# tanm-sys/forge-ec

Hardware: AMD Instinct MI355X
Metric: secp256k1-var scalar-muls/sec (batched, bit-exact vs CPU oracle on the parity sample) (higher is better)
Workload: dtype u32

## Files before the change

### forge_ec_amd/build.py

```python
import hashlib
import os
import subprocess
import sys

HERE = os.path.dirname(os.path.abspath(__file__))
SRC_DIR = os.path.join(HERE, "csrc")
OBJ_DIR = os.path.join(SRC_DIR, "_obj")
SO = os.path.join(HERE, "libfecgpu.so")
STAMP = SO + ".sha256"
SOURCES = ["fecgpu.hip", "canon.hip", "kernels_p256.hip", "kernels_ed.hip", "kernels_secp.hip", "kernels_codec.hip", "kernels_ecdsa.hip"]
HEADERS = ["coop.hpp", "sched_lf.hpp", "limbs.hpp", "staging.hpp", "host_ctx.hpp", "secp256k1.hpp", "p256.hpp", "ed25519.hpp",
           "canon_curves.hpp", "canon_kernels.hpp", "field_asm.inc", "kernels.hpp", "cu_split.hpp", os.path.join("..", "..", "include", "fecgpu.h"),
           os.path.join("..", "..", "include", "fecgpu_canon.h")]
FLAGS = ["--offload-arch=gfx950", "-O3", "-std=c++17", "-fPIC"]


def source_hash():
    h = hashlib.sha256(" ".join(FLAGS).encode())
    for rel in SOURCES + HEADERS:
        with open(os.path.join(SRC_DIR, rel), "rb") as f:
            h.update(rel.encode() + b"\0" + f.read())
    return h.hexdigest()


def up_to_date():
    try:
        return os.path.exists(SO) and open(STAMP).read().strip() == source_hash()
    except OSError:
        return False


DECLARATION_ONLY = ("kernels.hpp",)


def tu_closure_hash(src, kernel_code_only=False):
    import re
    seen, todo = [], [src]
    while todo:
        rel = todo.pop()
        if rel in seen or not os.path.exists(os.path.join(SRC_DIR, rel)) or (kernel_code_only and rel in DECLARATION_ONLY):
            continue
        seen.append(rel)
        with open(os.path.join(SRC_DIR, rel), "r") as f:
            todo += re.findall(r'^\s*#\s*include\s+"([^"/]+)"', f.read(), flags=re.M)
    h = hashlib.sha256(" ".join(FLAGS).encode())
    for rel in sorted(seen):
        with open(os.path.join(SRC_DIR, rel), "rb") as f:
            h.update(rel.encode() + b"\0" + f.read())
    return h.hexdigest()


WORKLOAD_TU = {"secp256k1-var": "kernels_secp.hip", "secp256k1-fixed": "kernels_secp.hip",
               "p256-var": "kernels_p256.hip", "p256-fixed": "kernels_p256.hip",
               "ed25519-var": "kernels_ed.hip", "ed25519-fixed": "kernels_ed.hip", "secp256k1-double": "kernels_secp.hip"}


def _tu_hash(src):
    return tu_closure_hash(src)


def build(force=False, verbose=False):
    if not force and up_to_date():
        return SO
    hipcc = os.environ.get("HIPCC", "/opt/rocm/bin/hipcc")
    os.makedirs(OBJ_DIR, exist_ok=True)
    for stale in (SO, STAMP):
        if os.path.exists(stale):
            os.remove(stale)
    jobs, objs, stamps = [], [], []
    for src in SOURCES:
        obj = os.path.join(OBJ_DIR, src.replace(".hip", ".o"))
        objs.append(obj)
        ostamp, want = obj + ".sha256", _tu_hash(src)
        try:
            if not force and os.path.exists(obj) and open(ostamp).read().strip() == want:
                continue
        except OSError:
            pass
        if os.path.exists(ostamp):
            os.remove(ostamp)
        cmd = [hipcc] + FLAGS + ["-c", os.path.join(SRC_DIR, src), "-o", obj]
        if verbose:
            print(" ".join(cmd), flush=True)
        jobs.append((cmd, subprocess.Popen(cmd)))
        stamps.append((ostamp, want))
    failed = [(cmd, proc.returncode) for cmd, proc in jobs if proc.wait() != 0]
    if failed:
        raise subprocess.CalledProcessError(failed[0][1], failed[0][0])
    for ostamp, want in stamps:
        with open(ostamp, "w") as f:
            f.write(want + "\n")
    cmd = [hipcc, "--offload-arch=gfx950", "-shared", "-fPIC", "-o", SO] + objs
    if verbose:
        print(" ".join(cmd), flush=True)
    subprocess.check_call(cmd)
    with open(STAMP, "w") as f:
        f.write(source_hash() + "\n")
    return SO


if __name__ == "__main__":
    print(build(force="--force" in sys.argv, verbose=True))
```

### forge_ec_amd/csrc/kernels_secp.hip

```cpp
#include <hip/hip_runtime.h>

#include "../../include/fecgpu.h"
#include "secp256k1.hpp"
#include "staging.hpp"
#include "kernels.hpp"

namespace fecgpu {

namespace {

FEC_DEV secp::pt ld3(const u32* l, int stride) {
  secp::pt p;
  FEC_UNROLL for (int i = 0; i < 8; ++i) {
    p.x.w[i] = l[i * stride];
    p.y.w[i] = l[(8 + i) * stride];
    p.z.w[i] = l[(16 + i) * stride];
  }
  return p;
}
FEC_DEV void st3(u32* l, int stride, const secp::pt& p) {
  FEC_UNROLL for (int i = 0; i < 8; ++i) {
    l[i * stride] = p.x.w[i];
    l[(8 + i) * stride] = p.y.w[i];
    l[(16 + i) * stride] = p.z.w[i];
  }
}

FEC_DEV fe ldc(const u32* l, int c) {
  fe a;
  FEC_UNROLL for (int i = 0; i < 8; ++i) a.w[i] = l[(8 * c + i) * TPB];
  return a;
}

FEC_DEV secp::pt padd_slots(const u32* lp, const u32* lq, lmask& need_double) {
  using namespace secp;
  fe z1s, z1c, z2s, z2c;
  lmask maybe;
  {
    const fe z1 = ldc(lp, 2);
    maybe = lanes_where(z1.w[0] == 0u);
    z1s = sqr(z1);
    z1c = mul(z1s, z1);
  }
  __builtin_amdgcn_sched_barrier(0);
  {
    const fe z2 = ldc(lq, 2);
    maybe |= lanes_where(z2.w[0] == 0u);
    z2s = sqr(z2);
    z2c = mul(z2s, z2);
  }
  __builtin_amdgcn_sched_barrier(0);
  const fe u1 = mul(ldc(lp, 0), z2s);
  const fe u2 = mul(ldc(lq, 0), z1s);
  __builtin_amdgcn_sched_barrier(0);
  const fe s1 = mul(ldc(lp, 1), z2c);
  const fe s2 = mul(ldc(lq, 1), z1c);
  __builtin_amdgcn_sched_barrier(0);
  lmask ueq = 0, seq = 0;
  if (__builtin_expect(lanes_where(u1.w[0] == u2.w[0]) != 0, 0)) {
    ueq = fe_eq(u1, u2);
    seq = fe_eq(s1, s2);
  }
  const fe h = sub(u2, u1);
  const fe r = sub(s2, s1);
  const fe h2 = sqr(h);
  const fe h3 = mul(h2, h);
  const fe u1h2 = mul(u1, h2);
  pt o;
  o.x = sub(sub(sub(sqr(r), h3), u1h2), u1h2);
  o.y = sub(mul(r, sub(u1h2, o.x)), mul(s1, h3));
  o.z = mul(mul(h, ldc(lp, 2)), ldc(lq, 2));
  need_double = 0;
  if (__builtin_expect((maybe | ueq) != 0, 0)) {
    const pt p = ld3(lp, TPB), q = ld3(lq, TPB);
    const lmask idp = is_identity(p), idq = is_identity(q);
    o = pt_select(o, identity(), ueq & ~seq);
    o = pt_select(o, p, idq);
    o = pt_select(o, q, idp);
    need_double = ueq & seq & ~idp & ~idq;
  }
  return o;
}

}

template <int MODE>
__global__ __launch_bounds__(TPB, 3) void k_secp_mul(const u32* __restrict__ scalars,
                                                  const u32* __restrict__ points,
                                                  u32* __restrict__ out, size_t n,
                                                  const u32* __restrict__ prefix, int wbits) {
  __shared__ u32 lds[48 * TPB];
  const int valid = block_valid(n);
  const size_t first = (size_t)blockIdx.x * TPB;
  const int e = threadIdx.x;
  if (MODE == 0) stage_in<24>(lds, points + first * 24, valid);
  __syncthreads();
  if (e < valid) {
    const size_t g = first + e;
    const u32* kg = scalars + g * 8;
    lmask early = 0;
    u32* const slot0 = lds + e;
    int i0 = 0, i1 = 256;
    if (MODE != 3) {
      u32 any = 0;
      FEC_UNROLL for (int i = 0; i < 8; ++i) any |= kg[i];
      early = lanes_where(any == 0);
    }
    if (MODE == 2) early |= secp::is_identity(ld3(points, 1));
    if (MODE == 2 || MODE == 3) {
      const u32 idx = MODE == 3 ? (u32)(g >> 1) : __builtin_bswap32(kg[0]) >> (32 - wbits);
      const uint4* row = reinterpret_cast<const uint4*>(prefix + (size_t)idx * 48);
      FEC_UNROLL for (int q = 0; q < 12; ++q) {
        const uint4 x = row[q];
        slot0[(4 * q + 0) * TPB] = x.x;
        slot0[(4 * q + 1) * TPB] = x.y;
        slot0[(4 * q + 2) * TPB] = x.z;
        slot0[(4 * q + 3) * TPB] = x.w;
      }
      i0 = MODE == 3 ? 0 : wbits;
      if (MODE == 3) i1 = 1;
    } else {
      const secp::pt r1 = MODE != 0 ? ld3(points, 1) : ld3(lds + e, TPB);
      early |= secp::is_identity(r1);
      st3(slot0, TPB, secp::identity());
      st3(slot0 + 24 * TPB, TPB, r1);
    }
    u32 kword = MODE == 3 ? 0u : kg[i0 >> 5];
#pragma unroll 1
    for (int i = i0; i < i1; ++i) {
      u32 b;
      if (MODE == 3) {
        b = (u32)g & 1u;
      } else {
        if ((i & 31) == 0) kword = kg[i >> 5];
        const int sh = (((i >> 3) & 3) << 3) + 7 - (i & 7);
        b = (kword >> sh) & 1u;
      }
      lmask nd;
      secp::pt s = padd_slots(slot0, slot0 + 24 * TPB, nd);
      if (__builtin_expect(nd != 0, 0)) {
        secp::pt d0 = secp::pdouble(ld3(slot0, TPB));
        s = secp::pt_select(s, d0, nd);
      }
      u32* const slot_d = slot0 + b * (24u * TPB);
      u32* const slot_s = slot0 + (b ^ 1u) * (24u * TPB);
      const secp::pt din = ld3(slot_d, TPB);
      st3(slot_s, TPB, s);
      st3(slot_d, TPB, secp::pdouble(din));
    }
    if (MODE != 3) {
      const secp::pt r0 = secp::pt_select(ld3(slot0, TPB), secp::identity(), early);
      st3(slot0, TPB, r0);
    }
  }
  __syncthreads();
  if (MODE == 3) stage_out<48>(out + first * 48, lds, valid);
  else stage_out<24>(out + first * 24, lds, valid);
}

void secp_launch_mul(const SchedEnv& env, bool fixed, const u32* scalars, const u32* points, u32* out, size_t n, hipStream_t s) {
  const unsigned grid = (unsigned)((n + TPB - 1) / TPB);
  const int w = (int)env.gen_prefix_bits[FEC_SECP256K1];
  if (fixed && w > 0 && points == env.gen[FEC_SECP256K1] && env.gen_prefix[FEC_SECP256K1] != nullptr)
    hipLaunchKernelGGL((k_secp_mul<2>), dim3(grid), dim3(TPB), 0, s, scalars, points, out, n, env.gen_prefix[FEC_SECP256K1], w);
  else if (fixed) hipLaunchKernelGGL((k_secp_mul<1>), dim3(grid), dim3(TPB), 0, s, scalars, points, out, n, (const u32*)nullptr, 0);
  else hipLaunchKernelGGL((k_secp_mul<0>), dim3(grid), dim3(TPB), 0, s, scalars, points, out, n, (const u32*)nullptr, 0);
}

void secp_prefix_level_launch(const u32* parent, u32* child, size_t child_entries, hipStream_t s) {
  hipLaunchKernelGGL((k_secp_mul<3>), dim3((unsigned)((child_entries + TPB - 1) / TPB)), dim3(TPB), 0, s, (const u32*)nullptr,
                     (const u32*)nullptr, child, child_entries, parent, 0);
}

}
```

### forge_ec_amd/csrc/secp256k1.hpp

```cpp
#pragma once
#include "limbs.hpp"

namespace fecgpu {
namespace secp {

#define FEC_SECP_C 0x3d1, 1, 0, 0, 0, 0, 0, 0
#define FEC_SECP_P 0xfffffc2f, -2, -1, -1, -1, -1, -1, -1

FEC_DEV fe csub_p(const fe& v) {
  fe w;
  lmask ov;
  FEC_ADDK256(w, v, ov, FEC_SECP_C);
  return fe_select(v, w, ov);
}
FEC_DEV lmask maybe_ge_p(const fe& v) {
  u32 ones = v.w[2] & v.w[3] & v.w[4] & v.w[5] & v.w[6] & v.w[7];
  return lanes_where(ones == 0xFFFFFFFFu);
}
FEC_DEV fe csub_p_unlikely(const fe& v) {
  if (__builtin_expect(maybe_ge_p(v) != 0, 0)) return csub_p(v);
  return v;
}

FEC_DEV fe add(const fe& a, const fe& b) {
  fe s;
  const lmask carry = add256(s, a, b);
  if (__builtin_expect(lanes_where(s.w[7] == 0xFFFFFFFFu) != 0, 0)) {
    fe w;
    lmask ov;
    FEC_ADDK256(w, s, ov, FEC_SECP_C);
    return fe_select(s, w, carry | ov);
  }
  lmask cy;
  FEC_ADD_SHORT2(s, carry, cy, 0x3d1);
  if (__builtin_expect(cy != 0, 0)) carry_from<2>(s, cy);
  return s;
}

FEC_DEV fe dbl(const fe& a) {
  fe s;
  const lmask carry = dbl256(s, a);
  if (__builtin_expect(lanes_where(s.w[7] == 0xFFFFFFFFu) != 0, 0)) {
    fe w;
    lmask ov;
    FEC_ADDK256(w, s, ov, FEC_SECP_C);
    return fe_select(s, w, carry | ov);
  }
  lmask cy;
  FEC_ADD_SHORT2(s, carry, cy, 0x3d1);
  if (__builtin_expect(cy != 0, 0)) carry_from<2>(s, cy);
  return s;
}

FEC_DEV fe sub(const fe& a, const fe& b) {
  fe d;
  const lmask borrow = sub256(d, a, b);
  lmask bw;
  FEC_SUB_SHORT2(d, borrow, bw, 0x3d1);
  if (__builtin_expect(bw != 0, 0)) borrow_from<2>(d, bw);
  return d;
}

FEC_DEV fe neg(const fe& a) {
  fe r;
  lmask t;
  FEC_KSUB256(r, a, t, FEC_SECP_P);
  (void)t;
  return fe_select(r, a, fe_is_zero(a));
}

FEC_DEV fe mont_reduce(const u32 t[16]) {
  const u32 N0P = 0xD2253531u;
  u32 m[8];
  u32 e_lo = 0, e_hi = 0;
  FEC_UNROLL for (int k = 0; k < 8; ++k) {
    u32 x = t[k] - e_lo;
    m[k] = x * N0P;
    u64 d = (u64)m[k] * 977u + (((u64)e_hi << 32) | e_lo);
    u64 e = (d >> 32) + m[k];
    e_lo = (u32)e;
    e_hi = (u32)(e >> 32);
  }
  fe th, mm, v, v2;
  FEC_UNROLL for (int i = 0; i < 8; ++i) {
    th.w[i] = t[8 + i];
    mm.w[i] = m[i];
  }
  add256(v, th, mm);
  sub_lohi256(v2, v, e_lo, e_hi);
  return csub_p_unlikely(v2);
}

FEC_DEV fe mul_small_cxx(const fe& a, u32 k) {
  u32 t[16];
  mul_wide_small(t, a, k);
  return mont_reduce(t);
}

FEC_DEV fe mul_cxx(const fe& a, const fe& b) {
  u32 t[16];
  mul_wide(t, a, b);
  return mont_reduce(t);
}

#ifdef FEC_HOST_EMUL
FEC_DEV fe mul(const fe& a, const fe& b) { return mul_cxx(a, b); }
#else
FEC_DEV fe borrow_from_word2(const fe& v, lmask bw) {
  fe x = v;
  asm("s_mov_b64 vcc, %6\n\t"
      "v_subbrev_co_u32_e32 %0, vcc, 0, %0, vcc\n\t"
      "v_subbrev_co_u32_e32 %1, vcc, 0, %1, vcc\n\t"
      "v_subbrev_co_u32_e32 %2, vcc, 0, %2, vcc\n\t"
      "v_subbrev_co_u32_e32 %3, vcc, 0, %3, vcc\n\t"
      "v_subbrev_co_u32_e32 %4, vcc, 0, %4, vcc\n\t"
      "v_subbrev_co_u32_e32 %5, vcc, 0, %5, vcc"
      : "+v"(x.w[2]), "+v"(x.w[3]), "+v"(x.w[4]), "+v"(x.w[5]), "+v"(x.w[6]), "+v"(x.w[7])
      : "s"(bw)
      : "vcc");
  return x;
}
FEC_DEV fe csub_p_top(const fe& v) {
  if (__builtin_expect(lanes_where(v.w[7] == 0xFFFFFFFFu) != 0, 0)) return csub_p_unlikely(v);
  return v;
}
FEC_DEV fe mul(const fe& a, const fe& b) {
  fe r;
  lmask sc, bw;
  asm(FEC_SECP_MUL_ASM
      : "=v"(r.w[0]), "=v"(r.w[1]), "=v"(r.w[2]), "=v"(r.w[3]), "=v"(r.w[4]), "=v"(r.w[5]), "=v"(r.w[6]),
        "=v"(r.w[7]), "=&s"(sc), "=&s"(bw)
      : FEC_V8(a), FEC_V8(b), "s"(0xD2253531u), "s"(977u)
      : FEC_SECP_MUL_CLOBBERS);
  if (__builtin_expect(bw != 0, 0)) r = borrow_from_word2(r, bw);
  return csub_p_top(r);
}
template <u32 K>
FEC_DEV fe mul_small_k(const fe& a) {
  static_assert(K == 3 || K == 8, "the ladder multiplies by 3 and 8 only");
  fe r;
  lmask sc, bw, exc;
  if (K == 3) {
    asm(FEC_SECP_MUL3_ASM
        : "=v"(r.w[0]), "=v"(r.w[1]), "=v"(r.w[2]), "=v"(r.w[3]), "=v"(r.w[4]), "=v"(r.w[5]), "=v"(r.w[6]),
          "=v"(r.w[7]), "=&s"(sc), "=&s"(bw), "=&s"(exc)
        : FEC_V8(a), "s"(0xD2253531u), "s"(977u)
        : FEC_SECP_MUL3_CLOBBERS);
  } else {
    asm(FEC_SECP_MUL8_ASM
        : "=v"(r.w[0]), "=v"(r.w[1]), "=v"(r.w[2]), "=v"(r.w[3]), "=v"(r.w[4]), "=v"(r.w[5]), "=v"(r.w[6]),
          "=v"(r.w[7]), "=&s"(sc), "=&s"(bw), "=&s"(exc)
        : FEC_V8(a), "s"(0xD2253531u), "s"(977u)
        : FEC_SECP_MUL8_CLOBBERS);
  }
  if (__builtin_expect(exc != 0, 0)) r = fe_select(r, mul_small_cxx(a, K), ~(lmask)0);
  else if (__builtin_expect(bw != 0, 0)) r = borrow_from_word2(r, bw);
  return csub_p_top(r);
}
#endif
#ifdef FEC_HOST_EMUL
FEC_DEV fe mul_small(const fe& a, u32 k) { return mul_small_cxx(a, k); }
#else
FEC_DEV fe mul_small(const fe& a, u32 k) { return k == 3 ? mul_small_k<3>(a) : (k == 8 ? mul_small_k<8>(a) : mul_small_cxx(a, k)); }
#endif


#ifdef FEC_HOST_EMUL
static unsigned long fec_host_rare_sqr = 0;
FEC_DEV lmask cross_add(u32& w0, u32& w1, u32& w2, u32& w3, u32& w4, u32& w5, u32 x0, u32 x1, u32 x2, u32 x3) {
  u64 lo = ((u64)w1 << 32) | w0, hi = ((u64)w3 << 32) | w2, nx = ((u64)w5 << 32) | w4;
  u64 xl = ((u64)x1 << 32) | x0, xh = ((u64)x3 << 32) | x2;
  u64 s0 = lo + xl, s1 = hi + xh;
  u64 inc = (s0 < xl) | (s1 < xh);
  u64 n2 = nx + inc;
  w0 = (u32)s0; w1 = (u32)(s0 >> 32); w2 = (u32)s1; w3 = (u32)(s1 >> 32); w4 = (u32)n2; w5 = (u32)(n2 >> 32);
  return (n2 < inc) ? ~0ull : 0ull;
}
FEC_DEV lmask fold_add(u32& r0, u32& r1, u32& r2, u32& r3, u32 m0, u32 m1) {
  u64 l0 = ((u64)r1 << 32) | r0, l1 = ((u64)r3 << 32) | r2, m = ((u64)m1 << 32) | m0;
  u64 t = l0 + m;
  u64 c = t < m;
  u64 t1 = l1 + c;
  r0 = (u32)t; r1 = (u32)(t >> 32); r2 = (u32)t1; r3 = (u32)(t1 >> 32);
  return (t1 < c) ? ~0ull : 0ull;
}
FEC_DEV lmask ripple2(u32& a, u32& b, lmask cin) {
  u64 v = ((u64)b << 32) | a, c = cin ? 1 : 0;
  u64 n = v + c;
  a = (u32)n; b = (u32)(n >> 32);
  return (n < c) ? ~0ull : 0ull;
}
#else
FEC_DEV lmask cross_add(u32& w0, u32& w1, u32& w2, u32& w3, u32& w4, u32& w5, u32 x0, u32 x1, u32 x2, u32 x3) {
  lmask more;
  asm("v_add_co_u32_e32 %0, vcc, %0, %7\n\t"
      "v_addc_co_u32_e32 %1, vcc, %1, %8, vcc\n\t"
      "s_mov_b64 %6, vcc\n\t"
      "v_add_co_u32_e32 %2, vcc, %2, %9\n\t"
      "v_addc_co_u32_e32 %3, vcc, %3, %10, vcc\n\t"
      "s_or_b64 vcc, vcc, %6\n\t"
      "v_addc_co_u32_e32 %4, vcc, 0, %4, vcc\n\t"
      "v_addc_co_u32_e32 %5, vcc, 0, %5, vcc\n\t"
      "s_mov_b64 %6, vcc"
      : "+v"(w0), "+v"(w1), "+v"(w2), "+v"(w3), "+v"(w4), "+v"(w5), "=&s"(more)
      : "v"(x0), "v"(x1), "v"(x2), "v"(x3)
      : "vcc");
  return more;
}
FEC_DEV lmask fold_add(u32& r0, u32& r1, u32& r2, u32& r3, u32 m0, u32 m1) {
  lmask more;
  asm("v_add_co_u32_e32 %0, vcc, %0, %5\n\t"
      "v_addc_co_u32_e32 %1, vcc, %1, %6, vcc\n\t"
      "v_addc_co_u32_e32 %2, vcc, 0, %2, vcc\n\t"
      "v_addc_co_u32_e32 %3, vcc, 0, %3, vcc\n\t"
      "s_mov_b64 %4, vcc"
      : "+v"(r0), "+v"(r1), "+v"(r2), "+v"(r3), "=s"(more)
      : "v"(m0), "v"(m1)
      : "vcc");
  return more;
}
FEC_DEV lmask ripple2(u32& a, u32& b, lmask cin) {
  lmask cout;
  asm("s_mov_b64 vcc, %3\n\t"
      "v_addc_co_u32_e32 %0, vcc, 0, %0, vcc\n\t"
      "v_addc_co_u32_e32 %1, vcc, 0, %1, vcc\n\t"
      "s_mov_b64 %2, vcc"
      : "+v"(a), "+v"(b), "=s"(cout)
      : "s"(cin)
      : "vcc");
  return cout;
}
#endif

FEC_DEV lmask fold_general(u32 r[8], u32 m0, u32 m1, lmask cin) {
  u64 m = ((u64)m1 << 32) | m0;
  u64 carry = word_select(0u, 1u, cin);
  u64 res0 = ((u64)r[1] << 32) | r[0];
  u64 t = res0 + m;
  t = t + carry;
  carry = (u64)(t < m) | ((u64)(t < carry) & (u64)(m != 0));
  r[0] = (u32)t;
  r[1] = (u32)(t >> 32);
  lmask c = lanes_where(carry != 0);
  FEC_UNROLL for (int j = 1; j < 4; ++j) c = ripple2(r[2 * j], r[2 * j + 1], c);
  return c;
}

FEC_DEV fe sqr_cxx(const fe& a) {
  u32 w[16];
  FEC_UNROLL for (int i = 0; i < 4; ++i)
      mul64_words(&w[4 * i], a.w[2 * i], a.w[2 * i + 1], a.w[2 * i], a.w[2 * i + 1]);
  FEC_UNROLL for (int i = 0; i < 4; ++i) {
    FEC_UNROLL for (int j = i + 1; j < 4; ++j) {
      u32 p[4];
      mul64_words(p, a.w[2 * i], a.w[2 * i + 1], a.w[2 * j], a.w[2 * j + 1]);
      u32 x0 = p[0] << 1;
      u32 x1 = (p[1] << 1) | (p[0] >> 31);
      u32 x2 = (p[2] << 1) | (p[1] >> 31);
      u32 x3 = (p[3] << 1) | (p[2] >> 31);
      const int B = 2 * (i + j);
      lmask more = cross_add(w[B], w[B + 1], w[B + 2], w[B + 3], w[B + 4], w[B + 5], x0, x1, x2, x3);
      if (B + 6 < 16) {
        if (__builtin_expect(more != 0, 0)) {
#ifdef FEC_HOST_EMUL
          ++fec_host_rare_sqr;
#endif
          FEC_UNROLL for (int k = B + 6; k < 16; k += 2) more = ripple2(w[k], w[k + 1], more);
        }
      }
    }
  }
  u32 r[8];
  FEC_UNROLL for (int i = 0; i < 8; ++i) r[i] = w[i];
  lmask carry = 0;
  FEC_UNROLL for (int i = 4; i < 8; ++i) {
    u32 h0 = w[2 * i], h1 = w[2 * i + 1];
    u64 q = (u64)h0 * 977u;
    u32 m0 = (u32)q;
    u32 m1 = (u32)(q >> 32) + h1 * 977u + h0;
    if (__builtin_expect(carry == 0, 1)) {
      lmask more = fold_add(r[0], r[1], r[2], r[3], m0, m1);
      if (__builtin_expect(more != 0, 0)) {
#ifdef FEC_HOST_EMUL
        ++fec_host_rare_sqr;
#endif
        more = ripple2(r[4], r[5], more);
        carry = ripple2(r[6], r[7], more);
      }
    } else {
#ifdef FEC_HOST_EMUL
      ++fec_host_rare_sqr;
#endif
      carry = fold_general(r, m0, m1, carry);
    }
  }
  fe o;
  FEC_UNROLL for (int i = 0; i < 8; ++i) o.w[i] = r[i];
  return csub_p_unlikely(o);
}

#ifdef FEC_HOST_EMUL
FEC_DEV fe sqr(const fe& a) { return sqr_cxx(a); }
#else
FEC_DEV fe sqr(const fe& a) {
  fe r;
  lmask tmp, exc;
  asm(FEC_SECP_SQR_ASM
      : "=v"(r.w[0]), "=v"(r.w[1]), "=v"(r.w[2]), "=v"(r.w[3]), "=&v"(r.w[4]), "=&v"(r.w[5]), "=&v"(r.w[6]),
        "=&v"(r.w[7]), "=&s"(tmp), "=&s"(exc)
      : FEC_V8(a), "s"(977u)
      : FEC_SECP_SQR_CLOBBERS);
  if (__builtin_expect(exc != 0, 0)) r = fe_select(r, sqr_cxx(a), ~(lmask)0);
  return csub_p_top(r);
}
#endif

struct pt {
  fe x, y, z;
};

FEC_DEV pt identity() {
  pt p;
  p.x = fe_zero();
  p.y = fe_small(1);
  p.z = fe_zero();
  return p;
}
FEC_DEV lmask is_identity(const pt& p) { return fe_is_zero(p.z); }

FEC_DEV pt pt_select(const pt& a, const pt& b, lmask choice) {
  pt r;
  r.x = fe_select(a.x, b.x, choice);
  r.y = fe_select(a.y, b.y, choice);
  r.z = fe_select(a.z, b.z, choice);
  return r;
}

FEC_DEV pt pdouble(const pt& p) {
  fe a = sqr(p.x);
  fe b = sqr(p.y);
  fe c = sqr(b);
  fe xpb2 = sqr(add(p.x, b));
  fe dd = sub(sub(xpb2, a), c);
  fe d = dbl(dd);
  fe e = mul_small(a, 3);
  fe f = sqr(e);
  pt r;
  r.x = sub(f, dbl(d));
  r.y = sub(mul(e, sub(d, r.x)), mul_small(c, 8));
  fe yz = mul(p.y, p.z);
  r.z = dbl(yz);
  lmask idp = is_identity(p);
  if (__builtin_expect(idp != 0, 0)) r = pt_select(r, identity(), idp);
  return r;
}

FEC_DEV pt padd_nodouble(const pt& p, const pt& q, lmask& need_double) {
  fe z1s = sqr(p.z);
  fe z2s = sqr(q.z);
  fe u1 = mul(p.x, z2s);
  fe u2 = mul(q.x, z1s);
  fe z1c = mul(z1s, p.z);
  fe z2c = mul(z2s, q.z);
  fe s1 = mul(p.y, z2c);
  fe s2 = mul(q.y, z1c);
  fe h = sub(u2, u1);
  fe r = sub(s2, s1);
  fe h2 = sqr(h);
  fe h3 = mul(h2, h);
  fe u1h2 = mul(u1, h2);
  pt o;
  o.x = sub(sub(sub(sqr(r), h3), u1h2), u1h2);
  o.y = sub(mul(r, sub(u1h2, o.x)), mul(s1, h3));
  o.z = mul(mul(h, p.z), q.z);
  lmask idp = is_identity(p), idq = is_identity(q);
  lmask ueq = fe_eq(u1, u2);
  need_double = 0;
  if (__builtin_expect((idp | idq | ueq) != 0, 0)) {
    lmask seq = fe_eq(s1, s2);
    o = pt_select(o, identity(), ueq & ~seq);
    o = pt_select(o, p, idq);
    o = pt_select(o, q, idp);
    need_double = ueq & seq & ~idp & ~idq;
  }
  return o;
}

FEC_DEV pt padd(const pt& p, const pt& q) {
  lmask nd;
  pt o = padd_nodouble(p, q, nd);
  if (nd != 0) {
    pt d = pdouble(p);
    o = pt_select(o, d, nd);
  }
  return o;
}

namespace coop {
enum { PX = 0, PY, PZ, QX, QY, QZ, Z1S, Z2S, U1, U2, Z1C, Z2C, S1, S2, H, R, H2, R2, H3, U1H2, HZ, T, S1H3, Z3, X3, DD, ONE, SLOTS };
constexpr int WORDS = SLOTS * 8;
#ifdef FEC_HOST_EMUL
FEC_DEV fe ld(const u32* sh, int slot) {
  fe a;
  FEC_UNROLL for (int i = 0; i < 8; ++i) a.w[i] = sh[slot * 8 + i];
  return a;
}
FEC_DEV void st(u32* sh, int slot, const fe& a) {
  FEC_UNROLL for (int i = 0; i < 8; ++i) sh[slot * 8 + i] = a.w[i];
}
#else
FEC_DEV fe ld(const u32* sh, int slot) {
  const uint4* s4 = reinterpret_cast<const uint4*>(sh + slot * 8);
  const uint4 lo = s4[0], hi = s4[1];
  fe a;
  a.w[0] = lo.x; a.w[1] = lo.y; a.w[2] = lo.z; a.w[3] = lo.w;
  a.w[4] = hi.x; a.w[5] = hi.y; a.w[6] = hi.z; a.w[7] = hi.w;
  return a;
}
FEC_DEV void st(u32* sh, int slot, const fe& a) {
  uint4* s4 = reinterpret_cast<uint4*>(sh + slot * 8);
  s4[0] = make_uint4(a.w[0], a.w[1], a.w[2], a.w[3]);
  s4[1] = make_uint4(a.w[4], a.w[5], a.w[6], a.w[7]);
}
#endif
#ifdef FEC_HOST_EMUL
FEC_DEV void sync() {}
FEC_DEV int lane_id() { return 0; }
#else
FEC_DEV void sync() {
  __builtin_amdgcn_fence(__ATOMIC_RELEASE, "wavefront");
  __builtin_amdgcn_wave_barrier();
  __builtin_amdgcn_fence(__ATOMIC_ACQUIRE, "wavefront");
}
FEC_DEV int lane_id() { return (int)(threadIdx.x & 63); }
#endif
FEC_DEV int pick(int lane, int a0, int a1, int a2, int a3) { return lane == 0 ? a0 : (lane == 1 ? a1 : (lane == 2 ? a2 : (lane == 3 ? a3 : ONE))); }
template <bool SQR>
FEC_DEV void level(u32* sh, int n, int a0, int a1, int a2, int a3, int b0, int b1, int b2, int b3, int o0, int o1, int o2, int o3) {
  const int lane = lane_id();
  const fe a = ld(sh, pick(lane, a0, a1, a2, a3));
  fe res;
  if (SQR) {
    res = sqr(a);
  } else {
    const fe b = ld(sh, pick(lane, b0, b1, b2, b3));
    res = mul(a, b);
  }
  if (lane < n) st(sh, pick(lane, o0, o1, o2, o3), res);
  sync();
}
}

FEC_DEV pt padd_coop(u32* sh) {
  using namespace coop;
#ifdef FEC_HOST_EMUL
  const pt p0 = {ld(sh, PX), ld(sh, PY), ld(sh, PZ)}, q0 = {ld(sh, QX), ld(sh, QY), ld(sh, QZ)};
  return padd(p0, q0);
#else
  const int lane = lane_id();
  level<true>(sh, 2, PZ, QZ, ONE, ONE, ONE, ONE, ONE, ONE, Z1S, Z2S, ONE, ONE);
  level<false>(sh, 4, PX, QX, Z1S, Z2S, Z2S, Z1S, PZ, QZ, U1, U2, Z1C, Z2C);
  level<false>(sh, 2, PY, QY, ONE, ONE, Z2C, Z1C, ONE, ONE, S1, S2, ONE, ONE);
  {
    const fe d = sub(ld(sh, pick(lane, U2, S2, ONE, ONE)), ld(sh, pick(lane, U1, S1, ONE, ONE)));
    const fe d2 = sqr(d);
    if (lane < 2) {
      st(sh, pick(lane, H, R, ONE, ONE), d);
      st(sh, pick(lane, H2, R2, ONE, ONE), d2);
    }
    sync();
  }
  level<false>(sh, 3, H2, U1, H, ONE, H, H2, PZ, ONE, H3, U1H2, HZ, ONE);
  pt o;
  {
    const fe h3 = ld(sh, H3), u1h2 = ld(sh, U1H2), r2 = ld(sh, R2);
    o.x = sub(sub(sub(r2, h3), u1h2), u1h2);
    const fe dd = sub(u1h2, o.x);
    const fe a = ld(sh, pick(lane, R, S1, HZ, ONE));
    const fe b = fe_select(ld(sh, pick(lane, ONE, H3, QZ, ONE)), dd, lanes_where(lane == 0));
    const fe res = mul(a, b);
    if (lane < 3) st(sh, pick(lane, T, S1H3, Z3, ONE), res);
    sync();
  }
  o.y = sub(ld(sh, T), ld(sh, S1H3));
  o.z = ld(sh, Z3);
  const fe u1 = ld(sh, U1), u2 = ld(sh, U2), s1 = ld(sh, S1), s2 = ld(sh, S2);
  const pt p = {ld(sh, PX), ld(sh, PY), ld(sh, PZ)}, q = {ld(sh, QX), ld(sh, QY), ld(sh, QZ)};
  const lmask idp = is_identity(p), idq = is_identity(q);
  const lmask ueq = fe_eq(u1, u2);
  if (__builtin_expect((idp | idq | ueq) != 0, 0)) {
    const lmask seq = fe_eq(s1, s2);
    o = pt_select(o, identity(), uniform_mask(ueq & ~seq));
    o = pt_select(o, p, idq);
    o = pt_select(o, q, idp);
    const lmask nd = uniform_mask(ueq & seq & ~idp & ~idq);
    if (nd != 0) o = pt_select(o, pdouble(p), nd);
  }
  return o;
#endif
}

FEC_DEV pt pdouble_trait(const pt& p) {
  fe xx = sqr(p.x);
  fe yy = sqr(p.y);
  fe yyyy = sqr(yy);
  fe xy2 = sqr(add(p.x, yy));
  fe w = sub(sub(xy2, xx), yyyy);
  fe d = add(w, w);
  fe e = mul_small(xx, 3);
  fe ee = sqr(e);
  pt r;
  r.x = sub(sub(ee, d), d);
  r.y = sub(mul(e, sub(d, r.x)), mul_small(yyyy, 8));
  fe z3 = add(p.y, p.y);
  r.z = fe_select(mul(z3, p.z), z3, fe_eq(p.z, fe_small(1)));
  return pt_select(r, identity(), is_identity(p));
}

FEC_DEV fe inv(const fe& a) {
  const u64 e[4] = {0xFFFFFFFEFFFFFC2DULL, 0xFFFFFFFFFFFFFFFFULL, 0xFFFFFFFFFFFFFFFFULL, 0xFFFFFFFFFFFFFFFFULL};
  fe result = fe_small(1);
#pragma unroll 1
  for (int i = 0; i < 4; ++i) {
#pragma unroll 1
    for (int j = 63; j >= 0; --j) {
      result = sqr(result);
      if ((e[i] >> j) & 1) result = mul(result, a);
    }
  }
  return fe_select(result, fe_zero(), fe_is_zero(a));
}

FEC_DEV lmask to_affine(const pt& p, fe& x, fe& y) {
  lmask inf = is_identity(p);
  fe zi = inv(p.z);
  fe zi2 = sqr(zi);
  fe zi3 = mul(zi2, zi);
  x = fe_select(mul(p.x, zi2), fe_zero(), inf);
  y = fe_select(mul(p.y, zi3), fe_zero(), inf);
  return inf;
}

FEC_DEV fe to_montgomery(const fe& a) {
  fe r2 = fe_zero();
  r2.w[0] = 0x000E9F61u; r2.w[2] = 0x07A20000u; r2.w[4] = 0x00000100u;
  return mul(a, r2);
}
FEC_DEV fe from_value(const fe& v, lmask& valid) {
  fe t;
  lmask ov;
  FEC_ADDK256(t, v, ov, FEC_SECP_C);
  valid = ~ov;
  return fe_select(fe_zero(), to_montgomery(v), uniform_mask(valid));
}
FEC_DEV fe pow_lsb(const fe& a, const u64 (&e)[4]) {
  fe result = fe_small(1), base = a;
#pragma unroll 1
  for (int w = 0; w < 4; ++w) {
#pragma unroll 1
    for (int j = 0; j < 64; ++j) {
      if ((e[w] >> j) & 1) result = mul(result, base);
      base = sqr(base);
    }
  }
  return result;
}
FEC_DEV fe sqrt_inherent(const fe& a, lmask& is_sqrt) {
  const u64 e[4] = {0xFF0CULL, 0xFFFFULL, 0xFFFEULL, 0x3FFFULL};
  fe s = pow_lsb(a, e);
  is_sqrt = fe_eq(sqr(s), a);
  return s;
}
FEC_DEV lmask affine_on_curve(const fe& x, const fe& y) {
  fe rhs = add(mul(sqr(x), x), to_montgomery(fe_small(7)));
  return fe_eq(sqr(y), rhs);
}
FEC_DEV lmask decompress(const fe& xv, lmask want_odd, fe& x, fe& y) {
  lmask valid;
  x = from_value(xv, valid);
  fe y2 = add(mul(sqr(x), x), fe_small(7));
  lmask is_sqrt;
  fe ye = sqrt_inherent(y2, is_sqrt);
  fe yo = neg(ye);
  fe red = mul(ye, fe_small(1));
  lmask parity = lanes_where((red.w[0] & 1u) != 0);
  y = fe_select(ye, yo, uniform_mask(want_odd ^ parity));
  return valid & is_sqrt & affine_on_curve(x, y);
}
FEC_DEV lmask decode_uncompressed(const fe& xv, const fe& yv, fe& x, fe& y) {
  lmask vx, vy;
  x = from_value(xv, vx);
  y = from_value(yv, vy);
  fe x3 = mul(mul(x, x), x);
  fe ax = mul(fe_zero(), x);
  fe rhs = add(add(x3, ax), fe_small(7));
  return vx & vy & fe_eq(mul(y, y), rhs) & affine_on_curve(x, y);
}

FEC_DEV u32 ladder_bit(const u32* kw, int i) {
  u32 w = kw[(i >> 5) * KSTRIDE];
  int sh = (((i >> 3) & 3) << 3) + 7 - (i & 7);
  return (w >> sh) & 1u;
}

FEC_DEV pt multiply(const pt& point, const u32* kw) {
  u32 any = 0;
  FEC_UNROLL for (int i = 0; i < 8; ++i) any |= kw[i * KSTRIDE];
  lmask early = is_identity(point) | lanes_where(any == 0);
  pt r0 = identity();
  pt r1 = point;
#pragma unroll 1
  for (int i = 0; i < 256; ++i) {
    lmask bit = lanes_where(ladder_bit(kw, i) != 0);
    lmask nd;
    pt s = padd_nodouble(r0, r1, nd);
    pt din = pt_select(r0, r1, bit);
    pt d;
#pragma unroll 1
    for (int pass = 0;; ++pass) {
      pt o = pdouble(din);
      if (pass == 0) {
        d = o;
        if (nd == 0) break;
        din = r0;
      } else {
        s = pt_select(s, o, nd);
        break;
      }
    }
    r0 = pt_select(d, s, bit);
    r1 = pt_select(s, d, bit);
  }
  return pt_select(r0, identity(), early);
}

FEC_DEV fe N_() {
  fe n;
  n.w[0] = 0xD0364141u; n.w[1] = 0xBFD25E8Cu; n.w[2] = 0xAF48A03Bu; n.w[3] = 0xBAAEDCE6u;
  n.w[4] = 0xFFFFFFFFu; n.w[5] = 0xFFFFFFFFu; n.w[6] = 0xFFFFFFFEu; n.w[7] = 0xFFFFFFFFu;
  return n;
}
FEC_DEV lmask sc_ge_n(const fe& a) {
  fe t;
  return ~sub256(t, a, N_());
}
FEC_DEV fe sc_reduce(const fe& a) {
  fe t;
  lmask borrow = sub256(t, a, N_());
  return fe_select(a, t, ~borrow);
}
FEC_DEV fe sc_mul(const fe& a, const fe& b) {
  u32 t[8];
  mul_low256(t, a, b);
  fe r;
  FEC_UNROLL for (int i = 0; i < 8; ++i) r.w[i] = t[i];
  return sc_reduce(r);
}
FEC_DEV fe sc_add(const fe& a, const fe& b) {
  fe t;
  (void)add256(t, a, b);
  return sc_reduce(t);
}
FEC_DEV fe sc_inv(const fe& a) {
  const u64 e[4] = {0xBFD25E8CD036413FULL, 0xBAAEDCE6AF48A03BULL, 0xFFFFFFFFFFFFFFFFULL, 0xFFFFFFFFFFFFFFFEULL};
  fe result = fe_small(1);
#pragma unroll 1
  for (int i = 0; i < 4; ++i) {
#pragma unroll 1
    for (int j = 63; j >= 0; --j) {
      result = sc_mul(result, result);
      if ((e[i] >> j) & 1) result = sc_mul(result, a);
    }
  }
  return result;
}

}
}
```

Before: 36.35 million.

## Add low-register-placement field asm variant and templated four-wave secp kernel

Adds a second copy of the secp256k1 mul/sqr/small-mul inline assembly whose scratch registers start at v92..v127 instead of the previous higher block. Field ops and pdouble are templated on the placement, and the kernel gains a FOUR template parameter chosen at launch when there are more than four waves per SIMD and the buffers don't alias badly. The aim is to cap VGPR usage so more waves fit per SIMD, at the cost of extra register pressure for the compiler around the asm blocks and more code to maintain.

```diff
diff --git a/forge_ec_amd/build.py b/forge_ec_amd/build.py
--- a/forge_ec_amd/build.py
+++ b/forge_ec_amd/build.py
@@ -10,7 +10,7 @@
 STAMP = SO + ".sha256"
 SOURCES = ["fecgpu.hip", "canon.hip", "kernels_p256.hip", "kernels_ed.hip", "kernels_secp.hip", "kernels_codec.hip", "kernels_ecdsa.hip"]
 HEADERS = ["coop.hpp", "sched_lf.hpp", "limbs.hpp", "staging.hpp", "host_ctx.hpp", "secp256k1.hpp", "p256.hpp", "ed25519.hpp",
-           "canon_curves.hpp", "canon_kernels.hpp", "field_asm.inc", "kernels.hpp", "cu_split.hpp", os.path.join("..", "..", "include", "fecgpu.h"),
+           "canon_curves.hpp", "canon_kernels.hpp", "field_asm.inc", "field_asm_ladder.inc", "kernels.hpp", "cu_split.hpp", os.path.join("..", "..", "include", "fecgpu.h"),
            os.path.join("..", "..", "include", "fecgpu_canon.h")]
 FLAGS = ["--offload-arch=gfx950", "-O3", "-std=c++17", "-fPIC"]
 
diff --git a/forge_ec_amd/csrc/field_asm_ladder.inc b/forge_ec_amd/csrc/field_asm_ladder.inc
--- /dev/null
+++ b/forge_ec_amd/csrc/field_asm_ladder.inc
@@ -0,0 +1,493 @@
+#pragma once
+
+#define FEC_SECP128_MUL_ASM \
+      "v_mov_b32_e32 v125, 0\n\t" \
+      "v_mov_b32_e32 v123, 0\n\t" \
+      "v_mad_u64_u32 v[92:93], vcc, %10, %18, 0\n\t" \
+      "v_mov_b32_e32 v122, v93\n\t" \
+      "v_mad_u64_u32 v[94:95], vcc, %10, %19, v[122:123]\n\t" \
+      "v_mad_u64_u32 v[94:95], vcc, %11, %18, v[94:95]\n\t" \
+      "v_addc_co_u32_e32 v123, vcc, 0, v123, vcc\n\t" \
+      "v_mul_lo_u32 v93, v92, %26\n\t" \
+      "v_mov_b32_e32 v122, v95\n\t" \
+      "v_mad_u64_u32 v[126:127], %9, v93, %27, 0\n\t" \
+      "v_add_co_u32_e64 v124, %8, v127, v93\n\t" \
+      "v_mad_u64_u32 v[96:97], vcc, %10, %20, v[122:123]\n\t" \
+      "v_addc_co_u32_e64 v123, vcc, 0, 0, vcc\n\t" \
+      "v_sub_u32_e32 v95, v94, v124\n\t" \
+      "v_mad_u64_u32 v[96:97], vcc, %11, %19, v[96:97]\n\t" \
+      "v_addc_co_u32_e32 v123, vcc, 0, v123, vcc\n\t" \
+      "v_mul_lo_u32 v95, v95, %26\n\t" \
+      "v_mad_u64_u32 v[96:97], vcc, %12, %18, v[96:97]\n\t" \
+      "v_addc_co_u32_e32 v123, vcc, 0, v123, vcc\n\t" \
+      "v_mad_u64_u32 v[126:127], %9, v95, %27, v[124:125]\n\t" \
+      "v_mov_b32_e32 v122, v97\n\t" \
+      "v_addc_co_u32_e64 v124, %8, v127, v95, %8\n\t" \
+      "v_mad_u64_u32 v[98:99], vcc, %10, %21, v[122:123]\n\t" \
+      "v_addc_co_u32_e64 v123, vcc, 0, 0, vcc\n\t" \
+      "v_sub_u32_e32 v97, v96, v124\n\t" \
+      "v_mad_u64_u32 v[98:99], vcc, %11, %20, v[98:99]\n\t" \
+      "v_addc_co_u32_e32 v123, vcc, 0, v123, vcc\n\t" \
+      "v_mul_lo_u32 v97, v97, %26\n\t" \
+      "v_mad_u64_u32 v[98:99], vcc, %12, %19, v[98:99]\n\t" \
+      "v_addc_co_u32_e32 v123, vcc, 0, v123, vcc\n\t" \
+      "v_mad_u64_u32 v[126:127], %9, v97, %27, v[124:125]\n\t" \
+      "v_mad_u64_u32 v[98:99], vcc, %13, %18, v[98:99]\n\t" \
+      "v_addc_co_u32_e32 v123, vcc, 0, v123, vcc\n\t" \
+      "v_addc_co_u32_e64 v124, %8, v127, v97, %8\n\t" \
+      "v_mov_b32_e32 v122, v99\n\t" \
+      "v_mad_u64_u32 v[100:101], vcc, %10, %22, v[122:123]\n\t" \
+      "v_addc_co_u32_e64 v123, vcc, 0, 0, vcc\n\t" \
+      "v_sub_u32_e32 v99, v98, v124\n\t" \
+      "v_mad_u64_u32 v[100:101], vcc, %11, %21, v[100:101]\n\t" \
+      "v_addc_co_u32_e32 v123, vcc, 0, v123, vcc\n\t" \
+      "v_mul_lo_u32 v99, v99, %26\n\t" \
+      "v_mad_u64_u32 v[100:101], vcc, %12, %20, v[100:101]\n\t" \
+      "v_addc_co_u32_e32 v123, vcc, 0, v123, vcc\n\t" \
+      "v_mad_u64_u32 v[126:127], %9, v99, %27, v[124:125]\n\t" \
+      "v_mad_u64_u32 v[100:101], vcc, %13, %19, v[100:101]\n\t" \
+      "v_addc_co_u32_e32 v123, vcc, 0, v123, vcc\n\t" \
+      "v_addc_co_u32_e64 v124, %8, v127, v99, %8\n\t" \
+      "v_mad_u64_u32 v[100:101], vcc, %14, %18, v[100:101]\n\t" \
+      "v_addc_co_u32_e32 v123, vcc, 0, v123, vcc\n\t" \
+      "v_mov_b32_e32 v122, v101\n\t" \
+      "v_mad_u64_u32 v[102:103], vcc, %10, %23, v[122:123]\n\t" \
+      "v_addc_co_u32_e64 v123, vcc, 0, 0, vcc\n\t" \
+      "v_sub_u32_e32 v101, v100, v124\n\t" \
+      "v_mad_u64_u32 v[102:103], vcc, %11, %22, v[102:103]\n\t" \
+      "v_addc_co_u32_e32 v123, vcc, 0, v123, vcc\n\t" \
+      "v_mul_lo_u32 v101, v101, %26\n\t" \
+      "v_mad_u64_u32 v[102:103], vcc, %12, %21, v[102:103]\n\t" \
+      "v_addc_co_u32_e32 v123, vcc, 0, v123, vcc\n\t" \
+      "v_mad_u64_u32 v[126:127], %9, v101, %27, v[124:125]\n\t" \
+      "v_mad_u64_u32 v[102:103], vcc, %13, %20, v[102:103]\n\t" \
+      "v_addc_co_u32_e32 v123, vcc, 0, v123, vcc\n\t" \
+      "v_addc_co_u32_e64 v124, %8, v127, v101, %8\n\t" \
+      "v_mad_u64_u32 v[102:103], vcc, %14, %19, v[102:103]\n\t" \
+      "v_addc_co_u32_e32 v123, vcc, 0, v123, vcc\n\t" \
+      "v_mad_u64_u32 v[102:103], vcc, %15, %18, v[102:103]\n\t" \
+      "v_addc_co_u32_e32 v123, vcc, 0, v123, vcc\n\t" \
+      "v_mov_b32_e32 v122, v103\n\t" \
+      "v_mad_u64_u32 v[104:105], vcc, %10, %24, v[122:123]\n\t" \
+      "v_addc_co_u32_e64 v123, vcc, 0, 0, vcc\n\t" \
+      "v_sub_u32_e32 v103, v102, v124\n\t" \
+      "v_mad_u64_u32 v[104:105], vcc, %11, %23, v[104:105]\n\t" \
+      "v_addc_co_u32_e32 v123, vcc, 0, v123, vcc\n\t" \
+      "v_mul_lo_u32 v103, v103, %26\n\t" \
+      "v_mad_u64_u32 v[104:105], vcc, %12, %22, v[104:105]\n\t" \
+      "v_addc_co_u32_e32 v123, vcc, 0, v123, vcc\n\t" \
+      "v_mad_u64_u32 v[126:127], %9, v103, %27, v[124:125]\n\t" \
+      "v_mad_u64_u32 v[104:105], vcc, %13, %21, v[104:105]\n\t" \
+      "v_addc_co_u32_e32 v123, vcc, 0, v123, vcc\n\t" \
+      "v_addc_co_u32_e64 v124, %8, v127, v103, %8\n\t" \
+      "v_mad_u64_u32 v[104:105], vcc, %14, %20, v[104:105]\n\t" \
+      "v_addc_co_u32_e32 v123, vcc, 0, v123, vcc\n\t" \
+      "v_mad_u64_u32 v[104:105], vcc, %15, %19, v[104:105]\n\t" \
+      "v_addc_co_u32_e32 v123, vcc, 0, v123, vcc\n\t" \
+      "v_mad_u64_u32 v[104:105], vcc, %16, %18, v[104:105]\n\t" \
+      "v_addc_co_u32_e32 v123, vcc, 0, v123, vcc\n\t" \
+      "v_mov_b32_e32 v122, v105\n\t" \
+      "v_mad_u64_u32 v[106:107], vcc, %10, %25, v[122:123]\n\t" \
+      "v_addc_co_u32_e64 v123, vcc, 0, 0, vcc\n\t" \
+      "v_sub_u32_e32 v105, v104, v124\n\t" \
+      "v_mad_u64_u32 v[106:107], vcc, %11, %24, v[106:107]\n\t" \
+      "v_addc_co_u32_e32 v123, vcc, 0, v123, vcc\n\t" \
+      "v_mul_lo_u32 v105, v105, %26\n\t" \
+      "v_mad_u64_u32 v[106:107], vcc, %12, %23, v[106:107]\n\t" \
+      "v_addc_co_u32_e32 v123, vcc, 0, v123, vcc\n\t" \
+      "v_mad_u64_u32 v[126:127], %9, v105, %27, v[124:125]\n\t" \
+      "v_mad_u64_u32 v[106:107], vcc, %13, %22, v[106:107]\n\t" \
+      "v_addc_co_u32_e32 v123, vcc, 0, v123, vcc\n\t" \
+      "v_addc_co_u32_e64 v124, %8, v127, v105, %8\n\t" \
+      "v_mad_u64_u32 v[106:107], vcc, %14, %21, v[106:107]\n\t" \
+      "v_addc_co_u32_e32 v123, vcc, 0, v123, vcc\n\t" \
+      "v_mad_u64_u32 v[106:107], vcc, %15, %20, v[106:107]\n\t" \
+      "v_addc_co_u32_e32 v123, vcc, 0, v123, vcc\n\t" \
+      "v_mad_u64_u32 v[106:107], vcc, %16, %19, v[106:107]\n\t" \
+      "v_addc_co_u32_e32 v123, vcc, 0, v123, vcc\n\t" \
+      "v_mad_u64_u32 v[106:107], vcc, %17, %18, v[106:107]\n\t" \
+      "v_addc_co_u32_e32 v123, vcc, 0, v123, vcc\n\t" \
+      "v_mov_b32_e32 v122, v107\n\t" \
+      "v_mad_u64_u32 v[108:109], vcc, %11, %25, v[122:123]\n\t" \
+      "v_addc_co_u32_e64 v123, vcc, 0, 0, vcc\n\t" \
+      "v_sub_u32_e32 v107, v106, v124\n\t" \
+      "v_mad_u64_u32 v[108:109], vcc, %12, %24, v[108:109]\n\t" \
+      "v_addc_co_u32_e32 v123, vcc, 0, v123, vcc\n\t" \
+      "v_mul_lo_u32 v107, v107, %26\n\t" \
+      "v_mad_u64_u32 v[108:109], vcc, %13, %23, v[108:109]\n\t" \
+      "v_addc_co_u32_e32 v123, vcc, 0, v123, vcc\n\t" \
+      "v_mad_u64_u32 v[126:127], %9, v107, %27, v[124:125]\n\t" \
+      "v_mad_u64_u32 v[108:109], vcc, %14, %22, v[108:109]\n\t" \
+      "v_addc_co_u32_e32 v123, vcc, 0, v123, vcc\n\t" \
+      "v_addc_co_u32_e64 v124, %8, v127, v107, %8\n\t" \
+      "v_mad_u64_u32 v[108:109], vcc, %15, %21, v[108:109]\n\t" \
+      "v_addc_co_u32_e32 v123, vcc, 0, v123, vcc\n\t" \
+      "v_mad_u64_u32 v[108:109], vcc, %16, %20, v[108:109]\n\t" \
+      "v_addc_co_u32_e32 v123, vcc, 0, v123, vcc\n\t" \
+      "v_mad_u64_u32 v[108:109], vcc, %17, %19, v[108:109]\n\t" \
+      "v_addc_co_u32_e32 v123, vcc, 0, v123, vcc\n\t" \
+      "v_mov_b32_e32 v122, v109\n\t" \
+      "v_mad_u64_u32 v[110:111], vcc, %12, %25, v[122:123]\n\t" \
+      "v_addc_co_u32_e64 v123, vcc, 0, 0, vcc\n\t" \
+      "v_mad_u64_u32 v[110:111], vcc, %13, %24, v[110:111]\n\t" \
+      "v_addc_co_u32_e32 v123, vcc, 0, v123, vcc\n\t" \
+      "v_mad_u64_u32 v[110:111], vcc, %14, %23, v[110:111]\n\t" \
+      "v_addc_co_u32_e32 v123, vcc, 0, v123, vcc\n\t" \
+      "v_mad_u64_u32 v[110:111], vcc, %15, %22, v[110:111]\n\t" \
+      "v_addc_co_u32_e32 v123, vcc, 0, v123, vcc\n\t" \
+      "v_mad_u64_u32 v[110:111], vcc, %16, %21, v[110:111]\n\t" \
+      "v_addc_co_u32_e32 v123, vcc, 0, v123, vcc\n\t" \
+      "v_mad_u64_u32 v[110:111], vcc, %17, %20, v[110:111]\n\t" \
+      "v_addc_co_u32_e32 v123, vcc, 0, v123, vcc\n\t" \
+      "v_mov_b32_e32 v122, v111\n\t" \
+      "v_mad_u64_u32 v[112:113], vcc, %13, %25, v[122:123]\n\t" \
+      "v_addc_co_u32_e64 v123, vcc, 0, 0, vcc\n\t" \
+      "v_mad_u64_u32 v[112:113], vcc, %14, %24, v[112:113]\n\t" \
+      "v_addc_co_u32_e32 v123, vcc, 0, v123, vcc\n\t" \
+      "v_mad_u64_u32 v[112:113], vcc, %15, %23, v[112:113]\n\t" \
+      "v_addc_co_u32_e32 v123, vcc, 0, v123, vcc\n\t" \
+      "v_mad_u64_u32 v[112:113], vcc, %16, %22, v[112:113]\n\t" \
+      "v_addc_co_u32_e32 v123, vcc, 0, v123, vcc\n\t" \
+      "v_mad_u64_u32 v[112:113], vcc, %17, %21, v[112:113]\n\t" \
+      "v_addc_co_u32_e32 v123, vcc, 0, v123, vcc\n\t" \
+      "v_mov_b32_e32 v122, v113\n\t" \
+      "v_mad_u64_u32 v[114:115], vcc, %14, %25, v[122:123]\n\t" \
+      "v_addc_co_u32_e64 v123, vcc, 0, 0, vcc\n\t" \
+      "v_mad_u64_u32 v[114:115], vcc, %15, %24, v[114:115]\n\t" \
+      "v_addc_co_u32_e32 v123, vcc, 0, v123, vcc\n\t" \
+      "v_mad_u64_u32 v[114:115], vcc, %16, %23, v[114:115]\n\t" \
+      "v_addc_co_u32_e32 v123, vcc, 0, v123, vcc\n\t" \
+      "v_mad_u64_u32 v[114:115], vcc, %17, %22, v[114:115]\n\t" \
+      "v_addc_co_u32_e32 v123, vcc, 0, v123, vcc\n\t" \
+      "v_mov_b32_e32 v122, v115\n\t" \
+      "v_mad_u64_u32 v[116:117], vcc, %15, %25, v[122:123]\n\t" \
+      "v_addc_co_u32_e64 v123, vcc, 0, 0, vcc\n\t" \
+      "v_mad_u64_u32 v[116:117], vcc, %16, %24, v[116:117]\n\t" \
+      "v_addc_co_u32_e32 v123, vcc, 0, v123, vcc\n\t" \
+      "v_mad_u64_u32 v[116:117], vcc, %17, %23, v[116:117]\n\t" \
+      "v_addc_co_u32_e32 v123, vcc, 0, v123, vcc\n\t" \
+      "v_mov_b32_e32 v122, v117\n\t" \
+      "v_mad_u64_u32 v[118:119], vcc, %16, %25, v[122:123]\n\t" \
+      "v_addc_co_u32_e64 v123, vcc, 0, 0, vcc\n\t" \
+      "v_mad_u64_u32 v[118:119], vcc, %17, %24, v[118:119]\n\t" \
+      "v_addc_co_u32_e32 v123, vcc, 0, v123, vcc\n\t" \
+      "v_mov_b32_e32 v122, v119\n\t" \
+      "v_mad_u64_u32 v[120:121], vcc, %17, %25, v[122:123]\n\t" \
+      "v_add_co_u32_e32 %0, vcc, v108, v93\n\t" \
+      "v_addc_co_u32_e32 %1, vcc, v110, v95, vcc\n\t" \
+      "v_addc_co_u32_e32 %2, vcc, v112, v97, vcc\n\t" \
+      "v_addc_co_u32_e32 %3, vcc, v114, v99, vcc\n\t" \
+      "v_addc_co_u32_e32 %4, vcc, v116, v101, vcc\n\t" \
+      "v_addc_co_u32_e32 %5, vcc, v118, v103, vcc\n\t" \
+      "v_addc_co_u32_e32 %6, vcc, v120, v105, vcc\n\t" \
+      "v_addc_co_u32_e32 %7, vcc, v121, v107, vcc\n\t" \
+      "v_cndmask_b32_e64 v125, 0, 1, %8\n\t" \
+      "v_sub_co_u32_e32 %0, vcc, %0, v124\n\t" \
+      "v_subb_co_u32_e32 %1, vcc, %1, v125, vcc\n\t" \
+      "s_mov_b64 %9, vcc"
+
+#define FEC_SECP128_MUL_CLOBBERS "vcc", "v92", "v93", "v94", "v95", "v96", "v97", "v98", "v99", "v100", "v101", "v102", "v103", "v104", "v105", "v106", "v107", "v108", "v109", "v110", "v111", "v112", "v113", "v114", "v115", "v116", "v117", "v118", "v119", "v120", "v121", "v122", "v123", "v124", "v125", "v126", "v127"
+
+
+#define FEC_SECP128_SQR_ASM \
+      "v_mov_b32_e32 v95, 0\n\t" \
+      "s_mov_b64 %9, 0\n\t" \
+      "v_mad_u64_u32 v[98:99], vcc, %10, %10, 0\n\t" \
+      "v_mov_b32_e32 v94, v99\n\t" \
+      "v_mad_u64_u32 v[100:101], vcc, %10, %11, v[94:95]\n\t" \
+      "v_mad_u64_u32 v[100:101], vcc, %11, %10, v[100:101]\n\t" \
+      "v_addc_co_u32_e64 v97, vcc, 0, 0, vcc\n\t" \
+      "v_mov_b32_e32 v96, v101\n\t" \
+      "v_mad_u64_u32 v[102:103], vcc, %11, %11, v[96:97]\n\t" \
+      "v_mad_u64_u32 v[104:105], vcc, %12, %12, 0\n\t" \
+      "v_mov_b32_e32 v94, v105\n\t" \
+      "v_mad_u64_u32 v[106:107], vcc, %12, %13, v[94:95]\n\t" \
+      "v_mad_u64_u32 v[106:107], vcc, %13, %12, v[106:107]\n\t" \
+      "v_addc_co_u32_e64 v97, vcc, 0, 0, vcc\n\t" \
+      "v_mov_b32_e32 v96, v107\n\t" \
+      "v_mad_u64_u32 v[108:109], vcc, %13, %13, v[96:97]\n\t" \
+      "v_mad_u64_u32 v[110:111], vcc, %14, %14, 0\n\t" \
+      "v_mov_b32_e32 v94, v111\n\t" \
+      "v_mad_u64_u32 v[112:113], vcc, %14, %15, v[94:95]\n\t" \
+      "v_mad_u64_u32 v[112:113], vcc, %15, %14, v[112:113]\n\t" \
+      "v_addc_co_u32_e64 v97, vcc, 0, 0, vcc\n\t" \
+      "v_mov_b32_e32 v96, v113\n\t" \
+      "v_mad_u64_u32 v[114:115], vcc, %15, %15, v[96:97]\n\t" \
+      "v_mad_u64_u32 v[116:117], vcc, %16, %16, 0\n\t" \
+      "v_mov_b32_e32 v94, v117\n\t" \
+      "v_mad_u64_u32 v[118:119], vcc, %16, %17, v[94:95]\n\t" \
+      "v_mad_u64_u32 v[118:119], vcc, %17, %16, v[118:119]\n\t" \
+      "v_addc_co_u32_e64 v97, vcc, 0, 0, vcc\n\t" \
+      "v_mov_b32_e32 v96, v119\n\t" \
+      "v_mad_u64_u32 v[120:121], vcc, %17, %17, v[96:97]\n\t" \
+      "v_mad_u64_u32 v[122:123], vcc, %10, %12, 0\n\t" \
+      "v_mov_b32_e32 v94, v123\n\t" \
+      "v_mad_u64_u32 v[124:125], vcc, %10, %13, v[94:95]\n\t" \
+      "v_mad_u64_u32 v[124:125], vcc, %11, %12, v[124:125]\n\t" \
+      "v_addc_co_u32_e64 v97, vcc, 0, 0, vcc\n\t" \
+      "v_mov_b32_e32 v96, v125\n\t" \
+      "v_mad_u64_u32 v[126:127], vcc, %11, %13, v[96:97]\n\t" \
+      "v_alignbit_b32 v127, v127, v126, 31\n\t" \
+      "v_alignbit_b32 v126, v126, v124, 31\n\t" \
+      "v_alignbit_b32 v124, v124, v122, 31\n\t" \
+      "v_lshlrev_b32_e32 v122, 1, v122\n\t" \
+      "v_add_co_u32_e32 v102, vcc, v102, v122\n\t" \
+      "v_addc_co_u32_e32 v103, vcc, v103, v124, vcc\n\t" \
+      "s_mov_b64 %8, vcc\n\t" \
+      "v_add_co_u32_e32 v104, vcc, v104, v126\n\t" \
+      "v_addc_co_u32_e32 v106, vcc, v106, v127, vcc\n\t" \
+      "s_or_b64 vcc, vcc, %8\n\t" \
+      "v_addc_co_u32_e32 v108, vcc, 0, v108, vcc\n\t" \
+      "v_addc_co_u32_e32 v109, vcc, 0, v109, vcc\n\t" \
+      "s_or_b64 %9, %9, vcc\n\t" \
+      "v_mad_u64_u32 v[122:123], vcc, %10, %14, 0\n\t" \
+      "v_mov_b32_e32 v94, v123\n\t" \
+      "v_mad_u64_u32 v[124:125], vcc, %10, %15, v[94:95]\n\t" \
+      "v_mad_u64_u32 v[124:125], vcc, %11, %14, v[124:125]\n\t" \
+      "v_addc_co_u32_e64 v97, vcc, 0, 0, vcc\n\t" \
+      "v_mov_b32_e32 v96, v125\n\t" \
+      "v_mad_u64_u32 v[126:127], vcc, %11, %15, v[96:97]\n\t" \
+      "v_alignbit_b32 v127, v127, v126, 31\n\t" \
+      "v_alignbit_b32 v126, v126, v124, 31\n\t" \
+      "v_alignbit_b32 v124, v124, v122, 31\n\t" \
+      "v_lshlrev_b32_e32 v122, 1, v122\n\t" \
+      "v_add_co_u32_e32 %4, vcc, v104, v122\n\t" \
+      "v_addc_co_u32_e32 %5, vcc, v106, v124, vcc\n\t" \
+      "s_mov_b64 %8, vcc\n\t" \
+      "v_add_co_u32_e32 v108, vcc, v108, v126\n\t" \
+      "v_addc_co_u32_e32 v109, vcc, v109, v127, vcc\n\t" \
+      "s_or_b64 vcc, vcc, %8\n\t" \
+      "v_addc_co_u32_e32 v110, vcc, 0, v110, vcc\n\t" \
+      "v_addc_co_u32_e32 v112, vcc, 0, v112, vcc\n\t" \
+      "s_or_b64 %9, %9, vcc\n\t" \
+      "v_mad_u64_u32 v[122:123], vcc, %10, %16, 0\n\t" \
+      "v_mov_b32_e32 v94, v123\n\t" \
+      "v_mad_u64_u32 v[124:125], vcc, %10, %17, v[94:95]\n\t" \
+      "v_mad_u64_u32 v[124:125], vcc, %11, %16, v[124:125]\n\t" \
+      "v_addc_co_u32_e64 v97, vcc, 0, 0, vcc\n\t" \
+      "v_mov_b32_e32 v96, v125\n\t" \
+      "v_mad_u64_u32 v[126:127], vcc, %11, %17, v[96:97]\n\t" \
+      "v_alignbit_b32 v127, v127, v126, 31\n\t" \
+      "v_alignbit_b32 v126, v126, v124, 31\n\t" \
+      "v_alignbit_b32 v124, v124, v122, 31\n\t" \
+      "v_lshlrev_b32_e32 v122, 1, v122\n\t" \
+      "v_add_co_u32_e32 v108, vcc, v108, v122\n\t" \
+      "v_addc_co_u32_e32 v109, vcc, v109, v124, vcc\n\t" \
+      "s_mov_b64 %8, vcc\n\t" \
+      "v_add_co_u32_e32 v110, vcc, v110, v126\n\t" \
+      "v_addc_co_u32_e32 v112, vcc, v112, v127, vcc\n\t" \
+      "s_or_b64 vcc, vcc, %8\n\t" \
+      "v_addc_co_u32_e32 v114, vcc, 0, v114, vcc\n\t" \
+      "v_addc_co_u32_e32 v115, vcc, 0, v115, vcc\n\t" \
+      "s_or_b64 %9, %9, vcc\n\t" \
+      "v_mad_u64_u32 v[122:123], vcc, %12, %14, 0\n\t" \
+      "v_mov_b32_e32 v94, v123\n\t" \
+      "v_mad_u64_u32 v[124:125], vcc, %12, %15, v[94:95]\n\t" \
+      "v_mad_u64_u32 v[124:125], vcc, %13, %14, v[124:125]\n\t" \
+      "v_addc_co_u32_e64 v97, vcc, 0, 0, vcc\n\t" \
+      "v_mov_b32_e32 v96, v125\n\t" \
+      "v_mad_u64_u32 v[126:127], vcc, %13, %15, v[96:97]\n\t" \
+      "v_alignbit_b32 v127, v127, v126, 31\n\t" \
+      "v_alignbit_b32 v126, v126, v124, 31\n\t" \
+      "v_alignbit_b32 v124, v124, v122, 31\n\t" \
+      "v_lshlrev_b32_e32 v122, 1, v122\n\t" \
+      "v_add_co_u32_e32 %6, vcc, v108, v122\n\t" \
+      "v_addc_co_u32_e32 %7, vcc, v109, v124, vcc\n\t" \
+      "s_mov_b64 %8, vcc\n\t" \
+      "v_add_co_u32_e32 v110, vcc, v110, v126\n\t" \
+      "v_addc_co_u32_e32 v112, vcc, v112, v127, vcc\n\t" \
+      "s_or_b64 vcc, vcc, %8\n\t" \
+      "v_addc_co_u32_e32 v114, vcc, 0, v114, vcc\n\t" \
+      "v_addc_co_u32_e32 v115, vcc, 0, v115, vcc\n\t" \
+      "s_or_b64 %9, %9, vcc\n\t" \
+      "v_mad_u64_u32 v[122:123], vcc, %12, %16, 0\n\t" \
+      "v_mov_b32_e32 v94, v123\n\t" \
+      "v_mad_u64_u32 v[124:125], vcc, %12, %17, v[94:95]\n\t" \
+      "v_mad_u64_u32 v[124:125], vcc, %13, %16, v[124:125]\n\t" \
+      "v_addc_co_u32_e64 v97, vcc, 0, 0, vcc\n\t" \
+      "v_mov_b32_e32 v96, v125\n\t" \
+      "v_mad_u64_u32 v[126:127], vcc, %13, %17, v[96:97]\n\t" \
+      "v_alignbit_b32 v127, v127, v126, 31\n\t" \
+      "v_alignbit_b32 v126, v126, v124, 31\n\t" \
+      "v_alignbit_b32 v124, v124, v122, 31\n\t" \
+      "v_lshlrev_b32_e32 v122, 1, v122\n\t" \
+      "v_add_co_u32_e32 v110, vcc, v110, v122\n\t" \
+      "v_addc_co_u32_e32 v112, vcc, v112, v124, vcc\n\t" \
+      "s_mov_b64 %8, vcc\n\t" \
+      "v_add_co_u32_e32 v114, vcc, v114, v126\n\t" \
+      "v_addc_co_u32_e32 v115, vcc, v115, v127, vcc\n\t" \
+      "s_or_b64 vcc, vcc, %8\n\t" \
+      "v_addc_co_u32_e32 v116, vcc, 0, v116, vcc\n\t" \
+      "v_addc_co_u32_e32 v118, vcc, 0, v118, vcc\n\t" \
+      "s_or_b64 %9, %9, vcc\n\t" \
+      "v_mad_u64_u32 v[122:123], vcc, %14, %16, 0\n\t" \
+      "v_mov_b32_e32 v94, v123\n\t" \
+      "v_mad_u64_u32 v[124:125], vcc, %14, %17, v[94:95]\n\t" \
+      "v_mad_u64_u32 v[124:125], vcc, %15, %16, v[124:125]\n\t" \
+      "v_addc_co_u32_e64 v97, vcc, 0, 0, vcc\n\t" \
+      "v_mov_b32_e32 v96, v125\n\t" \
+      "v_mad_u64_u32 v[126:127], vcc, %15, %17, v[96:97]\n\t" \
+      "v_alignbit_b32 v127, v127, v126, 31\n\t" \
+      "v_alignbit_b32 v126, v126, v124, 31\n\t" \
+      "v_alignbit_b32 v124, v124, v122, 31\n\t" \
+      "v_lshlrev_b32_e32 v122, 1, v122\n\t" \
+      "v_add_co_u32_e32 v114, vcc, v114, v122\n\t" \
+      "v_addc_co_u32_e32 v115, vcc, v115, v124, vcc\n\t" \
+      "s_mov_b64 %8, vcc\n\t" \
+      "v_add_co_u32_e32 v116, vcc, v116, v126\n\t" \
+      "v_addc_co_u32_e32 v118, vcc, v118, v127, vcc\n\t" \
+      "s_or_b64 vcc, vcc, %8\n\t" \
+      "v_addc_co_u32_e32 v120, vcc, 0, v120, vcc\n\t" \
+      "v_addc_co_u32_e32 v121, vcc, 0, v121, vcc\n\t" \
+      "v_mad_u64_u32 v[122:123], vcc, v110, %18, 0\n\t" \
+      "v_mul_lo_u32 v124, v112, %18\n\t" \
+      "v_add3_u32 v124, v123, v124, v110\n\t" \
+      "v_add_co_u32_e32 v98, vcc, v98, v122\n\t" \
+      "v_addc_co_u32_e32 v100, vcc, v100, v124, vcc\n\t" \
+      "v_addc_co_u32_e32 v102, vcc, 0, v102, vcc\n\t" \
+      "v_addc_co_u32_e32 v103, vcc, 0, v103, vcc\n\t" \
+      "s_or_b64 %9, %9, vcc\n\t" \
+      "v_mad_u64_u32 v[122:123], vcc, v114, %18, 0\n\t" \
+      "v_mul_lo_u32 v124, v115, %18\n\t" \
+      "v_add3_u32 v124, v123, v124, v114\n\t" \
+      "v_add_co_u32_e32 v98, vcc, v98, v122\n\t" \
+      "v_addc_co_u32_e32 v100, vcc, v100, v124, vcc\n\t" \
+      "v_addc_co_u32_e32 v102, vcc, 0, v102, vcc\n\t" \
+      "v_addc_co_u32_e32 v103, vcc, 0, v103, vcc\n\t" \
+      "s_or_b64 %9, %9, vcc\n\t" \
+      "v_mad_u64_u32 v[122:123], vcc, v116, %18, 0\n\t" \
+      "v_mul_lo_u32 v124, v118, %18\n\t" \
+      "v_add3_u32 v124, v123, v124, v116\n\t" \
+      "v_add_co_u32_e32 v98, vcc, v98, v122\n\t" \
+      "v_addc_co_u32_e32 v100, vcc, v100, v124, vcc\n\t" \
+      "v_addc_co_u32_e32 v102, vcc, 0, v102, vcc\n\t" \
+      "v_addc_co_u32_e32 v103, vcc, 0, v103, vcc\n\t" \
+      "s_or_b64 %9, %9, vcc\n\t" \
+      "v_mad_u64_u32 v[122:123], vcc, v120, %18, 0\n\t" \
+      "v_mul_lo_u32 v124, v121, %18\n\t" \
+      "v_add3_u32 v124, v123, v124, v120\n\t" \
+      "v_add_co_u32_e32 %0, vcc, v98, v122\n\t" \
+      "v_addc_co_u32_e32 %1, vcc, v100, v124, vcc\n\t" \
+      "v_addc_co_u32_e32 %2, vcc, 0, v102, vcc\n\t" \
+      "v_addc_co_u32_e32 %3, vcc, 0, v103, vcc\n\t" \
+      "s_or_b64 %9, %9, vcc"
+
+#define FEC_SECP128_SQR_CLOBBERS "vcc", "v94", "v95", "v96", "v97", "v98", "v99", "v100", "v101", "v102", "v103", "v104", "v105", "v106", "v107", "v108", "v109", "v110", "v111", "v112", "v113", "v114", "v115", "v116", "v117", "v118", "v119", "v120", "v121", "v122", "v123", "v124", "v125", "v126", "v127"
+
+
+#define FEC_SECP128_MUL3_ASM \
+      "v_mov_b32_e32 v123, 0\n\t" \
+      "v_mov_b32_e32 v125, 0\n\t" \
+      "v_mad_u64_u32 v[106:107], %9, %11, 3, 0\n\t" \
+      "v_mov_b32_e32 v122, v107\n\t" \
+      "v_mad_u64_u32 v[108:109], %9, %12, 3, v[122:123]\n\t" \
+      "v_mov_b32_e32 v122, v109\n\t" \
+      "v_mad_u64_u32 v[110:111], %9, %13, 3, v[122:123]\n\t" \
+      "v_mov_b32_e32 v122, v111\n\t" \
+      "v_mad_u64_u32 v[112:113], %9, %14, 3, v[122:123]\n\t" \
+      "v_mov_b32_e32 v122, v113\n\t" \
+      "v_mad_u64_u32 v[114:115], %9, %15, 3, v[122:123]\n\t" \
+      "v_mov_b32_e32 v122, v115\n\t" \
+      "v_mad_u64_u32 v[116:117], %9, %16, 3, v[122:123]\n\t" \
+      "v_mov_b32_e32 v122, v117\n\t" \
+      "v_mad_u64_u32 v[118:119], %9, %17, 3, v[122:123]\n\t" \
+      "v_mov_b32_e32 v122, v119\n\t" \
+      "v_mad_u64_u32 v[120:121], %9, %18, 3, v[122:123]\n\t" \
+      "v_mul_lo_u32 %0, v106, %19\n\t" \
+      "v_mad_u64_u32 v[126:127], %9, %0, %20, 0\n\t" \
+      "v_add_co_u32_e64 v124, %8, v127, %0\n\t" \
+      "v_sub_u32_e32 %1, v108, v124\n\t" \
+      "v_mul_lo_u32 %1, %1, %19\n\t" \
+      "v_mad_u64_u32 v[126:127], %9, %1, %20, v[124:125]\n\t" \
+      "v_addc_co_u32_e64 v124, %8, v127, %1, %8\n\t" \
+      "v_sub_u32_e32 %2, v110, v124\n\t" \
+      "v_mul_lo_u32 %2, %2, %19\n\t" \
+      "v_mad_u64_u32 v[126:127], %9, %2, %20, v[124:125]\n\t" \
+      "v_addc_co_u32_e64 v124, %8, v127, %2, %8\n\t" \
+      "v_sub_u32_e32 %3, v112, v124\n\t" \
+      "v_mul_lo_u32 %3, %3, %19\n\t" \
+      "v_mad_u64_u32 v[126:127], %9, %3, %20, v[124:125]\n\t" \
+      "v_addc_co_u32_e64 v124, %8, v127, %3, %8\n\t" \
+      "v_sub_u32_e32 %4, v114, v124\n\t" \
+      "v_mul_lo_u32 %4, %4, %19\n\t" \
+      "v_mad_u64_u32 v[126:127], %9, %4, %20, v[124:125]\n\t" \
+      "v_addc_co_u32_e64 v124, %8, v127, %4, %8\n\t" \
+      "v_sub_u32_e32 %5, v116, v124\n\t" \
+      "v_mul_lo_u32 %5, %5, %19\n\t" \
+      "v_mad_u64_u32 v[126:127], %9, %5, %20, v[124:125]\n\t" \
+      "v_addc_co_u32_e64 v124, %8, v127, %5, %8\n\t" \
+      "v_sub_u32_e32 %6, v118, v124\n\t" \
+      "v_mul_lo_u32 %6, %6, %19\n\t" \
+      "v_mad_u64_u32 v[126:127], %9, %6, %20, v[124:125]\n\t" \
+      "v_addc_co_u32_e64 v124, %8, v127, %6, %8\n\t" \
+      "v_sub_u32_e32 %7, v120, v124\n\t" \
+      "v_mul_lo_u32 %7, %7, %19\n\t" \
+      "v_mad_u64_u32 v[126:127], %9, %7, %20, v[124:125]\n\t" \
+      "v_addc_co_u32_e64 v124, %8, v127, %7, %8\n\t" \
+      "v_add_co_u32_e32 %0, vcc, %0, v121\n\t" \
+      "s_mov_b64 %10, vcc\n\t" \
+      "v_cndmask_b32_e64 v125, 0, 1, %8\n\t" \
+      "v_sub_co_u32_e32 %0, vcc, %0, v124\n\t" \
+      "v_subb_co_u32_e32 %1, vcc, %1, v125, vcc\n\t" \
+      "s_mov_b64 %9, vcc"
+
+#define FEC_SECP128_MUL3_CLOBBERS "vcc", "v106", "v107", "v108", "v109", "v110", "v111", "v112", "v113", "v114", "v115", "v116", "v117", "v118", "v119", "v120", "v121", "v122", "v123", "v124", "v125", "v126", "v127"
+
+
+#define FEC_SECP128_MUL8_ASM \
+      "v_mov_b32_e32 v123, 0\n\t" \
+      "v_mov_b32_e32 v125, 0\n\t" \
+      "v_mad_u64_u32 v[106:107], %9, %11, 8, 0\n\t" \
+      "v_mov_b32_e32 v122, v107\n\t" \
+      "v_mad_u64_u32 v[108:109], %9, %12, 8, v[122:123]\n\t" \
+      "v_mov_b32_e32 v122, v109\n\t" \
+      "v_mad_u64_u32 v[110:111], %9, %13, 8, v[122:123]\n\t" \
+      "v_mov_b32_e32 v122, v111\n\t" \
+      "v_mad_u64_u32 v[112:113], %9, %14, 8, v[122:123]\n\t" \
+      "v_mov_b32_e32 v122, v113\n\t" \
+      "v_mad_u64_u32 v[114:115], %9, %15, 8, v[122:123]\n\t" \
+      "v_mov_b32_e32 v122, v115\n\t" \
+      "v_mad_u64_u32 v[116:117], %9, %16, 8, v[122:123]\n\t" \
+      "v_mov_b32_e32 v122, v117\n\t" \
+      "v_mad_u64_u32 v[118:119], %9, %17, 8, v[122:123]\n\t" \
+      "v_mov_b32_e32 v122, v119\n\t" \
+      "v_mad_u64_u32 v[120:121], %9, %18, 8, v[122:123]\n\t" \
+      "v_mul_lo_u32 %0, v106, %19\n\t" \
+      "v_mad_u64_u32 v[126:127], %9, %0, %20, 0\n\t" \
+      "v_add_co_u32_e64 v124, %8, v127, %0\n\t" \
+      "v_sub_u32_e32 %1, v108, v124\n\t" \
+      "v_mul_lo_u32 %1, %1, %19\n\t" \
+      "v_mad_u64_u32 v[126:127], %9, %1, %20, v[124:125]\n\t" \
+      "v_addc_co_u32_e64 v124, %8, v127, %1, %8\n\t" \
+      "v_sub_u32_e32 %2, v110, v124\n\t" \
+      "v_mul_lo_u32 %2, %2, %19\n\t" \
+      "v_mad_u64_u32 v[126:127], %9, %2, %20, v[124:125]\n\t" \
+      "v_addc_co_u32_e64 v124, %8, v127, %2, %8\n\t" \
+      "v_sub_u32_e32 %3, v112, v124\n\t" \
+      "v_mul_lo_u32 %3, %3, %19\n\t" \
+      "v_mad_u64_u32 v[126:127], %9, %3, %20, v[124:125]\n\t" \
+      "v_addc_co_u32_e64 v124, %8, v127, %3, %8\n\t" \
+      "v_sub_u32_e32 %4, v114, v124\n\t" \
+      "v_mul_lo_u32 %4, %4, %19\n\t" \
+      "v_mad_u64_u32 v[126:127], %9, %4, %20, v[124:125]\n\t" \
+      "v_addc_co_u32_e64 v124, %8, v127, %4, %8\n\t" \
+      "v_sub_u32_e32 %5, v116, v124\n\t" \
+      "v_mul_lo_u32 %5, %5, %19\n\t" \
+      "v_mad_u64_u32 v[126:127], %9, %5, %20, v[124:125]\n\t" \
+      "v_addc_co_u32_e64 v124, %8, v127, %5, %8\n\t" \
+      "v_sub_u32_e32 %6, v118, v124\n\t" \
+      "v_mul_lo_u32 %6, %6, %19\n\t" \
+      "v_mad_u64_u32 v[126:127], %9, %6, %20, v[124:125]\n\t" \
+      "v_addc_co_u32_e64 v124, %8, v127, %6, %8\n\t" \
+      "v_sub_u32_e32 %7, v120, v124\n\t" \
+      "v_mul_lo_u32 %7, %7, %19\n\t" \
+      "v_mad_u64_u32 v[126:127], %9, %7, %20, v[124:125]\n\t" \
+      "v_addc_co_u32_e64 v124, %8, v127, %7, %8\n\t" \
+      "v_add_co_u32_e32 %0, vcc, %0, v121\n\t" \
+      "s_mov_b64 %10, vcc\n\t" \
+      "v_cndmask_b32_e64 v125, 0, 1, %8\n\t" \
+      "v_sub_co_u32_e32 %0, vcc, %0, v124\n\t" \
+      "v_subb_co_u32_e32 %1, vcc, %1, v125, vcc\n\t" \
+      "s_mov_b64 %9, vcc"
+
+#define FEC_SECP128_MUL8_CLOBBERS "vcc", "v106", "v107", "v108", "v109", "v110", "v111", "v112", "v113", "v114", "v115", "v116", "v117", "v118", "v119", "v120", "v121", "v122", "v123", "v124", "v125", "v126", "v127"
diff --git a/forge_ec_amd/csrc/kernels_secp.hip b/forge_ec_amd/csrc/kernels_secp.hip
--- a/forge_ec_amd/csrc/kernels_secp.hip
+++ b/forge_ec_amd/csrc/kernels_secp.hip
@@ -26,35 +26,94 @@
   }
 }
 
-FEC_DEV fe ldc(const u32* l, int c) {
-  fe a;
-  FEC_UNROLL for (int i = 0; i < 8; ++i) a.w[i] = l[(8 * c + i) * TPB];
-  return a;
-}
-
-FEC_DEV secp::pt padd_slots(const u32* lp, const u32* lq, lmask& need_double) {
+template <bool EXT>
+struct Ladder {
+  static constexpr int R1 = EXT ? 16 : 24;
+  static constexpr int LDS_WORDS = EXT ? 40 : 48;
+  u32* l;
+  __amdgpu_buffer_rsrc_t rsrc;
+  u32 voff, wstride;
+
+  FEC_DEV u32* slot(u32 b) const { return l + b * (u32)(R1 * TPB); }
+  FEC_DEV fe ld_x1() const {
+    if (!EXT) return load_fe(l + 24 * TPB, TPB);
+    fe x;
+    FEC_UNROLL for (int i = 0; i < 8; ++i) x.w[i] = __builtin_amdgcn_raw_buffer_load_b32(rsrc, voff, i * wstride, 0);
+    return x;
+  }
+  FEC_DEV void st_x1(const fe& x) const {
+    if (!EXT) return store_fe(l + 24 * TPB, TPB, x);
+    FEC_UNROLL for (int i = 0; i < 8; ++i) st_x1_word(i, x.w[i]);
+  }
+  FEC_DEV void st_x1_word(int i, u32 v) const { __builtin_amdgcn_raw_buffer_store_b32(v, rsrc, voff, i * wstride, 0); }
+  FEC_DEV void park(const secp::pt& p) const {
+    FEC_UNROLL for (int i = 0; i < 8; ++i) {
+      st_x1_word(8 + i, p.y.w[i]);
+      st_x1_word(16 + i, p.z.w[i]);
+    }
+  }
+  FEC_DEV void unpark(secp::pt& p) const {
+    FEC_UNROLL for (int i = 0; i < 8; ++i) {
+      p.y.w[i] = __builtin_amdgcn_raw_buffer_load_b32(rsrc, voff, (8 + i) * wstride, 0);
+      p.z.w[i] = __builtin_amdgcn_raw_buffer_load_b32(rsrc, voff, (16 + i) * wstride, 0);
+    }
+  }
+  FEC_DEV fe ldc(int s, int c) const { return s == 1 && c == 0 ? ld_x1() : load_fe(slot(s) + 8 * c * TPB, TPB); }
+  FEC_DEV secp::pt ld(int s) const {
+    secp::pt p;
+    p.x = ldc(s, 0);
+    p.y = ldc(s, 1);
+    p.z = ldc(s, 2);
+    return p;
+  }
+  FEC_DEV void st(int s, const secp::pt& p) const {
+    if (s == 1) st_x1(p.x);
+    else store_fe(l, TPB, p.x);
+    store_fe(slot(s) + 8 * TPB, TPB, p.y);
+    store_fe(slot(s) + 16 * TPB, TPB, p.z);
+  }
+  FEC_DEV secp::pt ld_sel(u32 b) const {
+    secp::pt p;
+    if (!EXT) p.x = load_fe(slot(b), TPB);
+    else if (b) p.x = ld_x1();
+    else p.x = load_fe(l, TPB);
+    p.y = load_fe(slot(b) + 8 * TPB, TPB);
+    p.z = load_fe(slot(b) + 16 * TPB, TPB);
+    return p;
+  }
+  FEC_DEV void st_sel(u32 b, const secp::pt& p) const {
+    if (!EXT) store_fe(slot(b), TPB, p.x);
+    else if (b) st_x1(p.x);
+    else store_fe(l, TPB, p.x);
+    store_fe(slot(b) + 8 * TPB, TPB, p.y);
+    store_fe(slot(b) + 16 * TPB, TPB, p.z);
+  }
+};
+
+template <int LT, bool EXT>
+FEC_DEV secp::pt padd_slots(const Ladder<EXT>& L, lmask& need_double) {
   using namespace secp;
   fe z1s, z1c, z2s, z2c;
   lmask maybe;
   {
-    const fe z1 = ldc(lp, 2);
+    const fe z1 = L.ldc(0, 2);
     maybe = lanes_where(z1.w[0] == 0u);
-    z1s = sqr(z1);
-    z1c = mul(z1s, z1);
+    z1s = sqr<LT>(z1);
+    z1c = mul<LT>(z1s, z1);
   }
   __builtin_amdgcn_sched_barrier(0);
   {
-    const fe z2 = ldc(lq, 2);
+    const fe z2 = L.ldc(1, 2);
     maybe |= lanes_where(z2.w[0] == 0u);
-    z2s = sqr(z2);
-    z2c = mul(z2s, z2);
-  }
-  __builtin_amdgcn_sched_barrier(0);
-  const fe u1 = mul(ldc(lp, 0), z2s);
-  const fe u2 = mul(ldc(lq, 0), z1s);
-  __builtin_amdgcn_sched_barrier(0);
-  const fe s1 = mul(ldc(lp, 1), z2c);
-  const fe s2 = mul(ldc(lq, 1), z1c);
+    z2s = sqr<LT>(z2);
+    z2c = mul<LT>(z2s, z2);
+  }
+  __builtin_amdgcn_sched_barrier(0);
+  const fe u1 = mul<LT>(L.ldc(0, 0), z2s);
+  const fe u2 = mul<LT>(L.ldc(1, 0), z1s);
+  __builtin_amdgcn_sched_barrier(0);
+  const fe s1 = mul<LT>(L.ldc(0, 1), z2c);
+  const fe s2 = mul<LT>(L.ldc(1, 1), z1c);
   __builtin_amdgcn_sched_barrier(0);
   lmask ueq = 0, seq = 0;
   if (__builtin_expect(lanes_where(u1.w[0] == u2.w[0]) != 0, 0)) {
@@ -63,16 +122,16 @@
   }
   const fe h = sub(u2, u1);
   const fe r = sub(s2, s1);
-  const fe h2 = sqr(h);
-  const fe h3 = mul(h2, h);
-  const fe u1h2 = mul(u1, h2);
+  const fe h2 = sqr<LT>(h);
+  const fe h3 = mul<LT>(h2, h);
+  const fe u1h2 = mul<LT>(u1, h2);
   pt o;
-  o.x = sub(sub(sub(sqr(r), h3), u1h2), u1h2);
-  o.y = sub(mul(r, sub(u1h2, o.x)), mul(s1, h3));
-  o.z = mul(mul(h, ldc(lp, 2)), ldc(lq, 2));
+  o.x = sub(sub(sub(sqr<LT>(r), h3), u1h2), u1h2);
+  o.y = sub(mul<LT>(r, sub(u1h2, o.x)), mul<LT>(s1, h3));
+  o.z = mul<LT>(mul<LT>(h, L.ldc(0, 2)), L.ldc(1, 2));
   need_double = 0;
   if (__builtin_expect((maybe | ueq) != 0, 0)) {
-    const pt p = ld3(lp, TPB), q = ld3(lq, TPB);
+    const pt p = L.ld(0), q = L.ld(1);
     const lmask idp = is_identity(p), idq = is_identity(q);
     o = pt_select(o, identity(), ueq & ~seq);
     o = pt_select(o, p, idq);
@@ -84,12 +143,16 @@
 
 }
 
-template <int MODE>
-__global__ __launch_bounds__(TPB, 3) void k_secp_mul(const u32* __restrict__ scalars,
-                                                  const u32* __restrict__ points,
-                                                  u32* __restrict__ out, size_t n,
-                                                  const u32* __restrict__ prefix, int wbits) {
-  __shared__ u32 lds[48 * TPB];
+template <int MODE, bool FOUR>
+__global__ __launch_bounds__(TPB, FOUR ? 4 : 3) void k_secp_mul(const u32* __restrict__ scalars,
+                                                                   const u32* __restrict__ points,
+                                                                   u32* __restrict__ out, size_t n,
+                                                                   const u32* __restrict__ prefix, int wbits) {
+  static_assert(MODE != 3 || !FOUR, "the table build keeps its 48-word entries in LDS");
+  constexpr bool EXT = FOUR;
+  constexpr int LT = FOUR ? secp::TOP_V128 : secp::TOP_V168;
+  using LD = Ladder<EXT>;
+  __shared__ u32 lds[LD::LDS_WORDS * TPB];
   const int valid = block_valid(n);
   const size_t first = (size_t)blockIdx.x * TPB;
   const int e = threadIdx.x;
@@ -99,7 +162,8 @@
     const size_t g = first + e;
     const u32* kg = scalars + g * 8;
     lmask early = 0;
-    u32* const slot0 = lds + e;
+    const LD L{lds + e, __builtin_amdgcn_make_buffer_rsrc(out + first * 24, 0, valid * 96, 0x00020000), (u32)e * 4u,
+               (u32)valid * 4u};
     int i0 = 0, i1 = 256;
     if (MODE != 3) {
       u32 any = 0;
@@ -112,18 +176,26 @@
       const uint4* row = reinterpret_cast<const uint4*>(prefix + (size_t)idx * 48);
       FEC_UNROLL for (int q = 0; q < 12; ++q) {
         const uint4 x = row[q];
-        slot0[(4 * q + 0) * TPB] = x.x;
-        slot0[(4 * q + 1) * TPB] = x.y;
-        slot0[(4 * q + 2) * TPB] = x.z;
-        slot0[(4 * q + 3) * TPB] = x.w;
+        if (EXT && (q == 6 || q == 7)) {
+          L.st_x1_word(4 * (q - 6) + 0, x.x);
+          L.st_x1_word(4 * (q - 6) + 1, x.y);
+          L.st_x1_word(4 * (q - 6) + 2, x.z);
+          L.st_x1_word(4 * (q - 6) + 3, x.w);
+          continue;
+        }
+        u32* const w = L.l + (EXT && q >= 8 ? 4 * q - 8 : 4 * q) * TPB;
+        w[0 * TPB] = x.x;
+        w[1 * TPB] = x.y;
+        w[2 * TPB] = x.z;
+        w[3 * TPB] = x.w;
       }
       i0 = MODE == 3 ? 0 : wbits;
       if (MODE == 3) i1 = 1;
     } else {
       const secp::pt r1 = MODE != 0 ? ld3(points, 1) : ld3(lds + e, TPB);
       early |= secp::is_identity(r1);
-      st3(slot0, TPB, secp::identity());
-      st3(slot0 + 24 * TPB, TPB, r1);
+      L.st(0, secp::identity());
+      L.st(1, r1);
     }
     u32 kword = MODE == 3 ? 0u : kg[i0 >> 5];
 #pragma unroll 1
@@ -137,20 +209,20 @@
         b = (kword >> sh) & 1u;
       }
       lmask nd;
-      secp::pt s = padd_slots(slot0, slot0 + 24 * TPB, nd);
+      secp::pt s = padd_slots<LT>(L, nd);
       if (__builtin_expect(nd != 0, 0)) {
-        secp::pt d0 = secp::pdouble(ld3(slot0, TPB));
+        if (EXT) L.park(s);
+        secp::pt d0 = secp::pdouble<LT>(L.ld(0));
+        if (EXT) L.unpark(s);
         s = secp::pt_select(s, d0, nd);
       }
-      u32* const slot_d = slot0 + b * (24u * TPB);
-      u32* const slot_s = slot0 + (b ^ 1u) * (24u * TPB);
-      const secp::pt din = ld3(slot_d, TPB);
-      st3(slot_s, TPB, s);
-      st3(slot_d, TPB, secp::pdouble(din));
+      const secp::pt din = L.ld_sel(b);
+      L.st_sel(b ^ 1u, s);
+      L.st_sel(b, secp::pdouble<LT>(din));
     }
     if (MODE != 3) {
-      const secp::pt r0 = secp::pt_select(ld3(slot0, TPB), secp::identity(), early);
-      st3(slot0, TPB, r0);
+      const secp::pt r0 = secp::pt_select(L.ld(0), secp::identity(), early);
+      L.st(0, r0);
     }
   }
   __syncthreads();
@@ -158,17 +230,27 @@
   else stage_out<24>(out + first * 24, lds, valid);
 }
 
-void secp_launch_mul(const SchedEnv& env, bool fixed, const u32* scalars, const u32* points, u32* out, size_t n, hipStream_t s) {
+template <bool FOUR>
+static void secp_launch_mul_t(const SchedEnv& env, bool fixed, const u32* scalars, const u32* points, u32* out, size_t n,
+                              hipStream_t s) {
   const unsigned grid = (unsigned)((n + TPB - 1) / TPB);
   const int w = (int)env.gen_prefix_bits[FEC_SECP256K1];
   if (fixed && w > 0 && points == env.gen[FEC_SECP256K1] && env.gen_prefix[FEC_SECP256K1] != nullptr)
-    hipLaunchKernelGGL((k_secp_mul<2>), dim3(grid), dim3(TPB), 0, s, scalars, points, out, n, env.gen_prefix[FEC_SECP256K1], w);
-  else if (fixed) hipLaunchKernelGGL((k_secp_mul<1>), dim3(grid), dim3(TPB), 0, s, scalars, points, out, n, (const u32*)nullptr, 0);
-  else hipLaunchKernelGGL((k_secp_mul<0>), dim3(grid), dim3(TPB), 0, s, scalars, points, out, n, (const u32*)nullptr, 0);
+    hipLaunchKernelGGL((k_secp_mul<2, FOUR>), dim3(grid), dim3(TPB), 0, s, scalars, points, out, n, env.gen_prefix[FEC_SECP256K1], w);
+  else if (fixed) hipLaunchKernelGGL((k_secp_mul<1, FOUR>), dim3(grid), dim3(TPB), 0, s, scalars, points, out, n, (const u32*)nullptr, 0);
+  else hipLaunchKernelGGL((k_secp_mul<0, FOUR>), dim3(grid), dim3(TPB), 0, s, scalars, points, out, n, (const u32*)nullptr, 0);
+}
+
+void secp_launch_mul(const SchedEnv& env, bool fixed, const u32* scalars, const u32* points, u32* out, size_t n, hipStream_t s) {
+  const size_t waves_per_simd = (n + 64 * 4 * (size_t)env.cus - 1) / (64 * 4 * (size_t)env.cus);
+  const size_t in_words = fixed ? 24 : n * 24;
+  const bool apart = out + n * 24 <= points || points + in_words <= out;
+  if (waves_per_simd > 4 && (apart || (!fixed && out == points))) secp_launch_mul_t<true>(env, fixed, scalars, points, out, n, s);
+  else secp_launch_mul_t<false>(env, fixed, scalars, points, out, n, s);
 }
 
 void secp_prefix_level_launch(const u32* parent, u32* child, size_t child_entries, hipStream_t s) {
-  hipLaunchKernelGGL((k_secp_mul<3>), dim3((unsigned)((child_entries + TPB - 1) / TPB)), dim3(TPB), 0, s, (const u32*)nullptr,
+  hipLaunchKernelGGL((k_secp_mul<3, false>), dim3((unsigned)((child_entries + TPB - 1) / TPB)), dim3(TPB), 0, s, (const u32*)nullptr,
                      (const u32*)nullptr, child, child_entries, parent, 0);
 }
 
diff --git a/forge_ec_amd/csrc/secp256k1.hpp b/forge_ec_amd/csrc/secp256k1.hpp
--- a/forge_ec_amd/csrc/secp256k1.hpp
+++ b/forge_ec_amd/csrc/secp256k1.hpp
@@ -1,11 +1,14 @@
 #pragma once
 #include "limbs.hpp"
+#include "field_asm_ladder.inc"
 
 namespace fecgpu {
 namespace secp {
 
 #define FEC_SECP_C 0x3d1, 1, 0, 0, 0, 0, 0, 0
 #define FEC_SECP_P 0xfffffc2f, -2, -1, -1, -1, -1, -1, -1
+
+constexpr int TOP_V168 = 168, TOP_V128 = 128;
 
 FEC_DEV fe csub_p(const fe& v) {
   fe w;
@@ -104,6 +107,7 @@
 }
 
 #ifdef FEC_HOST_EMUL
+template <int TOP = TOP_V168>
 FEC_DEV fe mul(const fe& a, const fe& b) { return mul_cxx(a, b); }
 #else
 FEC_DEV fe borrow_from_word2(const fe& v, lmask bw) {
@@ -124,34 +128,40 @@
   if (__builtin_expect(lanes_where(v.w[7] == 0xFFFFFFFFu) != 0, 0)) return csub_p_unlikely(v);
   return v;
 }
+#define FEC_SECP_MUL_STMT(NAME)                                                                                   \
+  asm(FEC_##NAME##_ASM                                                                                            \
+      : "=v"(r.w[0]), "=v"(r.w[1]), "=v"(r.w[2]), "=v"(r.w[3]), "=v"(r.w[4]), "=v"(r.w[5]), "=v"(r.w[6]),         \
+        "=v"(r.w[7]), "=&s"(sc), "=&s"(bw)                                                                        \
+      : FEC_V8(a), FEC_V8(b), "s"(0xD2253531u), "s"(977u)                                                         \
+      : FEC_##NAME##_CLOBBERS)
+template <int TOP = TOP_V168>
 FEC_DEV fe mul(const fe& a, const fe& b) {
+  static_assert(TOP == TOP_V168 || TOP == TOP_V128, "two placements of the blocks");
   fe r;
   lmask sc, bw;
-  asm(FEC_SECP_MUL_ASM
-      : "=v"(r.w[0]), "=v"(r.w[1]), "=v"(r.w[2]), "=v"(r.w[3]), "=v"(r.w[4]), "=v"(r.w[5]), "=v"(r.w[6]),
-        "=v"(r.w[7]), "=&s"(sc), "=&s"(bw)
-      : FEC_V8(a), FEC_V8(b), "s"(0xD2253531u), "s"(977u)
-      : FEC_SECP_MUL_CLOBBERS);
+  if constexpr (TOP == TOP_V128) FEC_SECP_MUL_STMT(SECP128_MUL);
+  else FEC_SECP_MUL_STMT(SECP_MUL);
   if (__builtin_expect(bw != 0, 0)) r = borrow_from_word2(r, bw);
   return csub_p_top(r);
 }
-template <u32 K>
+#define FEC_SECP_MUL_SMALL_STMT(NAME)                                                                             \
+  asm(FEC_##NAME##_ASM                                                                                            \
+      : "=v"(r.w[0]), "=v"(r.w[1]), "=v"(r.w[2]), "=v"(r.w[3]), "=v"(r.w[4]), "=v"(r.w[5]), "=v"(r.w[6]),         \
+        "=v"(r.w[7]), "=&s"(sc), "=&s"(bw), "=&s"(exc)                                                            \
+      : FEC_V8(a), "s"(0xD2253531u), "s"(977u)                                                                    \
+      : FEC_##NAME##_CLOBBERS)
+template <u32 K, int TOP = TOP_V168>
 FEC_DEV fe mul_small_k(const fe& a) {
   static_assert(K == 3 || K == 8, "the ladder multiplies by 3 and 8 only");
+  static_assert(TOP == TOP_V168 || TOP == TOP_V128, "two placements of the blocks");
   fe r;
   lmask sc, bw, exc;
-  if (K == 3) {
-    asm(FEC_SECP_MUL3_ASM
-        : "=v"(r.w[0]), "=v"(r.w[1]), "=v"(r.w[2]), "=v"(r.w[3]), "=v"(r.w[4]), "=v"(r.w[5]), "=v"(r.w[6]),
-          "=v"(r.w[7]), "=&s"(sc), "=&s"(bw), "=&s"(exc)
-        : FEC_V8(a), "s"(0xD2253531u), "s"(977u)
-        : FEC_SECP_MUL3_CLOBBERS);
+  if constexpr (TOP == TOP_V128) {
+    if constexpr (K == 3) FEC_SECP_MUL_SMALL_STMT(SECP128_MUL3);
+    else FEC_SECP_MUL_SMALL_STMT(SECP128_MUL8);
   } else {
-    asm(FEC_SECP_MUL8_ASM
-        : "=v"(r.w[0]), "=v"(r.w[1]), "=v"(r.w[2]), "=v"(r.w[3]), "=v"(r.w[4]), "=v"(r.w[5]), "=v"(r.w[6]),
-          "=v"(r.w[7]), "=&s"(sc), "=&s"(bw), "=&s"(exc)
-        : FEC_V8(a), "s"(0xD2253531u), "s"(977u)
-        : FEC_SECP_MUL8_CLOBBERS);
+    if constexpr (K == 3) FEC_SECP_MUL_SMALL_STMT(SECP_MUL3);
+    else FEC_SECP_MUL_SMALL_STMT(SECP_MUL8);
   }
   if (__builtin_expect(exc != 0, 0)) r = fe_select(r, mul_small_cxx(a, K), ~(lmask)0);
   else if (__builtin_expect(bw != 0, 0)) r = borrow_from_word2(r, bw);
@@ -159,9 +169,13 @@
 }
 #endif
 #ifdef FEC_HOST_EMUL
+template <int TOP = TOP_V168>
 FEC_DEV fe mul_small(const fe& a, u32 k) { return mul_small_cxx(a, k); }
 #else
-FEC_DEV fe mul_small(const fe& a, u32 k) { return k == 3 ? mul_small_k<3>(a) : (k == 8 ? mul_small_k<8>(a) : mul_small_cxx(a, k)); }
+template <int TOP = TOP_V168>
+FEC_DEV fe mul_small(const fe& a, u32 k) {
+  return k == 3 ? mul_small_k<3, TOP>(a) : (k == 8 ? mul_small_k<8, TOP>(a) : mul_small_cxx(a, k));
+}
 #endif
 
 
@@ -300,16 +314,22 @@
 }
 
 #ifdef FEC_HOST_EMUL
+template <int TOP = TOP_V168>
 FEC_DEV fe sqr(const fe& a) { return sqr_cxx(a); }
 #else
+#define FEC_SECP_SQR_STMT(NAME)                                                                                   \
+  asm(FEC_##NAME##_ASM                                                                                            \
+      : "=v"(r.w[0]), "=v"(r.w[1]), "=v"(r.w[2]), "=v"(r.w[3]), "=&v"(r.w[4]), "=&v"(r.w[5]), "=&v"(r.w[6]),      \
+        "=&v"(r.w[7]), "=&s"(tmp), "=&s"(exc)                                                                     \
+      : FEC_V8(a), "s"(977u)                                                                                      \
+      : FEC_##NAME##_CLOBBERS)
+template <int TOP = TOP_V168>
 FEC_DEV fe sqr(const fe& a) {
+  static_assert(TOP == TOP_V168 || TOP == TOP_V128, "two placements of the blocks");
   fe r;
   lmask tmp, exc;
-  asm(FEC_SECP_SQR_ASM
-      : "=v"(r.w[0]), "=v"(r.w[1]), "=v"(r.w[2]), "=v"(r.w[3]), "=&v"(r.w[4]), "=&v"(r.w[5]), "=&v"(r.w[6]),
-        "=&v"(r.w[7]), "=&s"(tmp), "=&s"(exc)
-      : FEC_V8(a), "s"(977u)
-      : FEC_SECP_SQR_CLOBBERS);
+  if constexpr (TOP == TOP_V128) FEC_SECP_SQR_STMT(SECP128_SQR);
+  else FEC_SECP_SQR_STMT(SECP_SQR);
   if (__builtin_expect(exc != 0, 0)) r = fe_select(r, sqr_cxx(a), ~(lmask)0);
   return csub_p_top(r);
 }
@@ -336,19 +356,20 @@
   return r;
 }
 
+template <int TOP = TOP_V168>
 FEC_DEV pt pdouble(const pt& p) {
-  fe a = sqr(p.x);
-  fe b = sqr(p.y);
-  fe c = sqr(b);
-  fe xpb2 = sqr(add(p.x, b));
+  fe a = sqr<TOP>(p.x);
+  fe b = sqr<TOP>(p.y);
+  fe c = sqr<TOP>(b);
+  fe xpb2 = sqr<TOP>(add(p.x, b));
   fe dd = sub(sub(xpb2, a), c);
   fe d = dbl(dd);
-  fe e = mul_small(a, 3);
-  fe f = sqr(e);
+  fe e = mul_small<TOP>(a, 3);
+  fe f = sqr<TOP>(e);
   pt r;
   r.x = sub(f, dbl(d));
-  r.y = sub(mul(e, sub(d, r.x)), mul_small(c, 8));
-  fe yz = mul(p.y, p.z);
+  r.y = sub(mul<TOP>(e, sub(d, r.x)), mul_small<TOP>(c, 8));
+  fe yz = mul<TOP>(p.y, p.z);
   r.z = dbl(yz);
   lmask idp = is_identity(p);
   if (__builtin_expect(idp != 0, 0)) r = pt_select(r, identity(), idp);
```

Result: no change. 36.62 million, median of 6 (+0.7%).
